# dimforge/salva

Hardware: AMD Instinct MI355X
Metric: particle-steps/sec (3D DFSPH) (higher is better)
Workload: dtype f32

## Files before the change

### bindings/rust/salva3d-hip/src/ffi.rs

```rust
#![allow(non_camel_case_types, non_snake_case, dead_code)]

#[repr(C)] pub struct SalvaHipWorld { _private: [u8; 0] }
#[repr(C)] pub struct SalvaHipComm { _private: [u8; 0] }
#[repr(C)] pub struct SalvaHipPeerSetup { _private: [u8; 0] }

pub const SALVA_HIP_OK: i32 = 0;
pub const SALVA_HIP_E_HIP: i32 = -1;
pub const SALVA_HIP_E_INVALID: i32 = -2;
pub const SALVA_HIP_E_NUMERIC: i32 = -3;
pub const SALVA_HIP_E_CAPACITY: i32 = -4;

pub const SALVA_HIP_SOLVER_DFSPH: i32 = 0;
pub const SALVA_HIP_SOLVER_IISPH: i32 = 1;

pub const SALVA_HIP_KERNEL_CUBIC_SPLINE: i32 = 0;
pub const SALVA_HIP_KERNEL_POLY6: i32 = 1;
pub const SALVA_HIP_KERNEL_SPIKY: i32 = 2;
pub const SALVA_HIP_KERNEL_VISCOSITY: i32 = 3;

pub const SALVA_HIP_FORCE_XSPH: i32 = 1;
pub const SALVA_HIP_FORCE_ARTIFICIAL: i32 = 2;
pub const SALVA_HIP_FORCE_AKINCI2013: i32 = 3;
pub const SALVA_HIP_FORCE_DFSPH_VISCOSITY: i32 = 4;
pub const SALVA_HIP_FORCE_HE2014: i32 = 5;
pub const SALVA_HIP_FORCE_WCSPH_TENSION: i32 = 6;
pub const SALVA_HIP_FORCE_CUSTOM: i32 = 7;
pub const SALVA_HIP_FORCE_BECKER2009: i32 = 8;
pub const SALVA_HIP_FORCE_DEVICE: i32 = 9;

pub const SALVA_HIP_DEVICE_NEEDS_FF: i32 = 1;
pub const SALVA_HIP_DEVICE_NEEDS_FB: i32 = 2;
pub const SALVA_HIP_DEVICE_NEEDS_KERNEL: i32 = 4;

pub const SALVA_HIP_DIRTY_POSITIONS: i32 = 1;
pub const SALVA_HIP_DIRTY_VELOCITIES: i32 = 2;
pub const SALVA_HIP_DIRTY_VOLUMES: i32 = 4;
pub const SALVA_HIP_DIRTY_ACCELERATIONS: i32 = 8;
pub const SALVA_HIP_DIRTY_ALL: i32 = 15;

pub const SALVA_HIP_FIELD_DENSITY: i32 = 0;
pub const SALVA_HIP_FIELD_ALPHA: i32 = 1;
pub const SALVA_HIP_FIELD_NUM_FLUID_CONTACTS: i32 = 2;
pub const SALVA_HIP_FIELD_NUM_BOUNDARY_CONTACTS: i32 = 3;
pub const SALVA_HIP_FIELD_VELOCITY_CHANGE: i32 = 4;
pub const SALVA_HIP_FIELD_PRESSURE: i32 = 5;
pub const SALVA_HIP_FIELD_VOLUME: i32 = 6;
pub const SALVA_HIP_FIELD_ACCELERATION: i32 = 7;

pub const SALVA_HIP_SHAPE_BALL: i32 = 1;
pub const SALVA_HIP_SHAPE_CUBOID: i32 = 2;
pub const SALVA_HIP_SHAPE_CAPSULE: i32 = 3;
pub const SALVA_HIP_SHAPE_CYLINDER: i32 = 4;
pub const SALVA_HIP_SHAPE_MESH: i32 = 5;
pub const SALVA_HIP_SHAPE_HOST: i32 = 100;

pub const SALVA_HIP_SAMPLE_SURFACE: i32 = 0;
pub const SALVA_HIP_SAMPLE_VOLUME: i32 = 1;

pub const SALVA_HIP_MESH_ORIENTED: i32 = 1;

pub const SALVA_HIP_SHAPE_COMPOUND: i32 = 6;

pub const SALVA_HIP_COMPOUND_MAX_PARTS: i32 = 64;

pub const SALVA_HIP_DEVICE_VIEW_VERSION: i32 = 1;
pub const SALVA_HIP_DEVICE_VIEW_BYTES: i32 = 240;
pub const SALVA_HIP_PEER_HANDLE_BYTES: i32 = 64;

#[repr(C)] #[derive(Clone, Copy, Debug)]
pub struct SalvaHipCounters_stages {
    pub collision_detection_time: f64,
    pub solver_time: f64,
}

#[repr(C)] #[derive(Clone, Copy, Debug)]
pub struct SalvaHipCounters_cd {
    pub ncontacts: u64,
    pub boundary_update_time: f64,
    pub grid_insertion_time: f64,
    pub neighborhood_search_time: f64,
    pub contact_sorting_time: f64,
}

#[repr(C)] #[derive(Clone, Copy, Debug)]
pub struct SalvaHipCounters_solver {
    pub non_pressure_resolution_time: f64,
    pub pressure_resolution_time: f64,
}

#[repr(C)] #[derive(Clone, Copy, Debug)]
pub struct SalvaHipParams {
    pub particle_radius: f32,
    pub smoothing_factor: f32,
    pub solver: i32,
    pub min_pressure_iter: i32,
    pub max_pressure_iter: i32,
    pub max_density_error: f32,
    pub min_divergence_iter: i32,
    pub max_divergence_iter: i32,
    pub max_divergence_error: f32,
    pub device: i32,
    pub enable_timers: i32,
    pub kernel_density: i32,
    pub kernel_gradient: i32,
    pub reserved: [i32; 5],
}

#[repr(C)] #[derive(Clone, Copy, Debug)]
pub struct SalvaHipForceDesc {
    pub kind: i32,
    pub p: [f32; 7],
}

#[repr(C)] #[derive(Clone, Copy, Debug)]
pub struct SalvaHipStepStats {
    pub n_divergence_iters: i32,
    pub n_pressure_iters: i32,
    pub divergence_error: f32,
    pub density_error: f32,
    pub ncontacts: u64,
    pub nparticles: u64,
    pub grid_ms: f32,
    pub solver_ms: f32,
    pub step_ms: f32,
    pub reserved: [f32; 5],
}

#[repr(C)] #[derive(Clone, Copy, Debug)]
pub struct SalvaHipCounters {
    pub nsubsteps: u64,
// ... 217 lines not shown
```

### include/salva_hip.h

```cpp
#ifndef SALVA_HIP_H
#define SALVA_HIP_H

#include <stdint.h>

#ifdef __cplusplus
extern "C" {
#endif

typedef struct SalvaHipWorld SalvaHipWorld;

enum {
    SALVA_HIP_OK = 0,
    SALVA_HIP_E_HIP = -1,
    SALVA_HIP_E_INVALID = -2,
    SALVA_HIP_E_NUMERIC = -3,
    SALVA_HIP_E_CAPACITY = -4
};

enum { SALVA_HIP_SOLVER_DFSPH = 0, SALVA_HIP_SOLVER_IISPH = 1 };
enum {
    SALVA_HIP_KERNEL_CUBIC_SPLINE = 0,
    SALVA_HIP_KERNEL_POLY6 = 1,
    SALVA_HIP_KERNEL_SPIKY = 2,
    SALVA_HIP_KERNEL_VISCOSITY = 3
// ... 16 lines not shown
    int32_t reserved[5];
} SalvaHipParams;

enum {
    SALVA_HIP_FORCE_XSPH = 1,
    SALVA_HIP_FORCE_ARTIFICIAL = 2,
    SALVA_HIP_FORCE_AKINCI2013 = 3,
    SALVA_HIP_FORCE_DFSPH_VISCOSITY = 4,
    SALVA_HIP_FORCE_HE2014 = 5,
    SALVA_HIP_FORCE_WCSPH_TENSION = 6,
    SALVA_HIP_FORCE_CUSTOM = 7,
    SALVA_HIP_FORCE_BECKER2009 = 8,
    SALVA_HIP_FORCE_DEVICE = 9
};
enum {
    SALVA_HIP_DEVICE_NEEDS_FF = 1,
    SALVA_HIP_DEVICE_NEEDS_FB = 2,
    SALVA_HIP_DEVICE_NEEDS_KERNEL = 4
};
typedef struct SalvaHipForceDesc {
    int32_t kind;
    float p[7];
} SalvaHipForceDesc;

enum {
    SALVA_HIP_DIRTY_POSITIONS = 1,
    SALVA_HIP_DIRTY_VELOCITIES = 2,
    SALVA_HIP_DIRTY_VOLUMES = 4,
    SALVA_HIP_DIRTY_ACCELERATIONS = 8,
    SALVA_HIP_DIRTY_ALL = 15
};

typedef struct SalvaHipStepStats {
    int32_t n_divergence_iters;
    int32_t n_pressure_iters;
    float divergence_error;
    float density_error;
    uint64_t ncontacts;
    uint64_t nparticles;
    float grid_ms;
    float solver_ms;
    float step_ms;
    float reserved[5];
} SalvaHipStepStats;

typedef struct SalvaHipCounters {
    uint64_t nsubsteps;
    double step_time;
    double custom;
    struct {
        double collision_detection_time;
        double solver_time;
    } stages;
    struct {
        uint64_t ncontacts;
        double boundary_update_time;
        double grid_insertion_time;
        double neighborhood_search_time;
        double contact_sorting_time;
    } cd;
    struct {
        double non_pressure_resolution_time;
        double pressure_resolution_time;
    } solver;
    int32_t n_divergence_iters, n_pressure_iters;
    uint64_t speculative_passes;
    uint64_t discarded_passes;
    uint64_t chained_passes;
    uint64_t chain_breaks;
    uint64_t pregrid_adopted;
    uint64_t pregrid_dropped;
    uint64_t light_class_passes;
    uint64_t sparse_class_passes;
} SalvaHipCounters;

enum {
    SALVA_HIP_FIELD_DENSITY = 0,
    SALVA_HIP_FIELD_ALPHA = 1,
    SALVA_HIP_FIELD_NUM_FLUID_CONTACTS = 2,
    SALVA_HIP_FIELD_NUM_BOUNDARY_CONTACTS = 3,
    SALVA_HIP_FIELD_VELOCITY_CHANGE = 4,
    SALVA_HIP_FIELD_PRESSURE = 5,
    SALVA_HIP_FIELD_VOLUME = 6,
    SALVA_HIP_FIELD_ACCELERATION = 7
};

void salva_hip_default_params(SalvaHipParams* out);

int salva_hip_create(const SalvaHipParams* params, SalvaHipWorld** out);
void salva_hip_destroy(SalvaHipWorld* world);

float salva_hip_h(const SalvaHipWorld* world);

int salva_hip_set_fluid(SalvaHipWorld* world, uint32_t slot, uint64_t n,
                        const float* positions_xyz, const float* velocities_xyz, const float* volumes,
                        const float* accelerations_xyz, const float* velocity_changes_xyz,
                        float density0, uint32_t memberships, uint32_t filter, uint32_t dirty_mask);

int salva_hip_set_fluid_forces(SalvaHipWorld* world, uint32_t slot, const SalvaHipForceDesc* forces, uint32_t nforces);

int salva_hip_remove_fluid(SalvaHipWorld* world, uint32_t slot);

int salva_hip_set_boundary(SalvaHipWorld* world, uint32_t slot, uint64_t n,
                           const float* positions_xyz, const float* velocities_xyz,
                           uint32_t memberships, uint32_t filter, int32_t wants_forces);
int salva_hip_remove_boundary(SalvaHipWorld* world, uint32_t slot);

uint32_t salva_hip_num_fluids(const SalvaHipWorld* world);
uint32_t salva_hip_num_boundaries(const SalvaHipWorld* world);
uint64_t salva_hip_fluid_len(const SalvaHipWorld* world, uint32_t slot);
uint64_t salva_hip_boundary_len(const SalvaHipWorld* world, uint32_t slot);

int salva_hip_step(SalvaHipWorld* world, float dt, const float gravity[3], SalvaHipStepStats* stats_or_null);

int salva_hip_get_fluid(SalvaHipWorld* world, uint32_t slot, float* positions_xyz, float* velocities_xyz);
int salva_hip_get_fluid_field(SalvaHipWorld* world, uint32_t slot, int32_t field, float* out);

typedef struct SalvaHipRigidPose {
    float translation[3];
    float rotation[4];
    float linvel[3];
    float angvel[3];
    float world_com[3];
    int32_t has_body;
    int32_t is_dynamic;
} SalvaHipRigidPose;

int salva_hip_set_boundary_sampling(SalvaHipWorld* world, uint32_t slot, uint64_t n, const float* local_points_xyz,
                                    uint32_t memberships, uint32_t filter);
int salva_hip_update_boundary_pose(SalvaHipWorld* world, uint32_t slot, const SalvaHipRigidPose* pose);
int salva_hip_update_boundary_poses(SalvaHipWorld* world, uint32_t n, const uint32_t* slots, const SalvaHipRigidPose* poses);
int salva_hip_get_boundary_particles(SalvaHipWorld* world, uint32_t slot, float* positions_xyz, float* velocities_xyz);
int salva_hip_get_boundary_wrench(SalvaHipWorld* world, uint32_t slot, const float point[3], float force[3], float torque[3]);
int salva_hip_get_boundary_wrenches(SalvaHipWorld* world, uint32_t n, const uint32_t* slots, const float* points_xyz, float* forces_xyz,
                                    float* torques_xyz);

typedef int (*SalvaHipForceCallback)(void* user, SalvaHipWorld* world, uint32_t fluid_slot, uint32_t force_index, float dt,
                                     float inv_dt);
int salva_hip_set_force_callback(SalvaHipWorld* world, SalvaHipForceCallback cb, void* user);
int salva_hip_force_get_state(SalvaHipWorld* world, uint32_t slot, float* positions_xyz, float* velocities_xyz, float* densities);
int salva_hip_force_add_accelerations(SalvaHipWorld* world, uint32_t slot, const float* accelerations_xyz);

#define SALVA_HIP_DEVICE_VIEW_VERSION 1
#define SALVA_HIP_DEVICE_VIEW_BYTES 240
typedef struct SalvaHipDeviceView {
    uint32_t struct_size;
    uint32_t version;
    void* stream;
    uint32_t fluid_slot, force_index;
    float dt, inv_dt;
    float h, particle_radius;
    int32_t kernel_density, kernel_gradient;
    float params[7];
    uint32_t needs;
    uint32_t n, nfluids;
    const float* posm;
    const float* vel;
    float* acc;
    const float* rho;
    const uint32_t* model;
    const uint32_t* id;
    const float* rho0;
    uint32_t nb;
    float bforce_scale;
    const float* bposv;
    const float* bvel;
    const uint32_t* bid;
// ... 192 lines not shown
```

### salva_amd/_lib.py

```python
from __future__ import annotations

import ctypes as C
import os
import subprocess

_HERE = os.path.dirname(os.path.abspath(__file__))
CSRC = os.path.join(_HERE, "csrc")
LIB_PATH = os.path.join(CSRC, "libsalva_hip.so")
if os.environ.get("SALVA_HIP_LIB_VARIANT"):
    LIB_PATH = os.path.join(CSRC, "libsalva_hip_%s.so" % os.environ["SALVA_HIP_LIB_VARIANT"])

OK, E_HIP, E_INVALID, E_NUMERIC, E_CAPACITY = 0, -1, -2, -3, -4
SOLVER_DFSPH, SOLVER_IISPH = 0, 1
(FORCE_XSPH, FORCE_ARTIFICIAL, FORCE_AKINCI2013, FORCE_DFSPH_VISCOSITY, FORCE_HE2014, FORCE_WCSPH_TENSION, FORCE_CUSTOM,
 FORCE_BECKER2009, FORCE_DEVICE) = 1, 2, 3, 4, 5, 6, 7, 8, 9
DEVICE_NEEDS_FF, DEVICE_NEEDS_FB, DEVICE_NEEDS_KERNEL = 1, 2, 4
DIRTY_POSITIONS, DIRTY_VELOCITIES, DIRTY_VOLUMES, DIRTY_ACCELERATIONS, DIRTY_ALL = 1, 2, 4, 8, 15
(FIELD_DENSITY, FIELD_ALPHA, FIELD_NUM_FLUID_CONTACTS, FIELD_NUM_BOUNDARY_CONTACTS, FIELD_VELOCITY_CHANGE,
 FIELD_PRESSURE, FIELD_VOLUME, FIELD_ACCELERATION) = range(8)

EXPORTED_SYMBOLS = [
    "salva_hip_default_params", "salva_hip_create", "salva_hip_destroy", "salva_hip_h", "salva_hip_set_fluid",
    "salva_hip_set_fluid_forces", "salva_hip_remove_fluid", "salva_hip_set_boundary", "salva_hip_remove_boundary",
    "salva_hip_num_fluids", "salva_hip_num_boundaries", "salva_hip_fluid_len", "salva_hip_boundary_len",
    "salva_hip_step", "salva_hip_get_fluid", "salva_hip_get_fluid_field", "salva_hip_get_boundary",
    "salva_hip_clear_boundary_forces", "salva_hip_device_bytes", "salva_hip_time_pred_density",
    "salva_hip_last_error", "salva_hip_version", "salva_hip_comm_rccl_unique_id", "salva_hip_comm_rccl_create",
    "salva_hip_comm_loopback_create", "salva_hip_comm_destroy", "salva_hip_set_domain", "salva_hip_get_owned",
    "salva_hip_get_force_stats", "salva_hip_get_fluid_contacts", "salva_hip_add_particles", "salva_hip_delete_particles",
    "salva_hip_particles_intersecting_aabb", "salva_hip_set_boundary_sampling", "salva_hip_update_boundary_pose",
    "salva_hip_get_boundary_particles", "salva_hip_get_boundary_wrench", "salva_hip_set_force_callback",
    "salva_hip_force_get_state", "salva_hip_force_add_accelerations", "salva_hip_set_fluid_field", "salva_hip_get_timestep",
    "salva_hip_set_timestep", "salva_hip_get_counters", "salva_hip_time_kernel", "salva_hip_particles_intersecting_shape", "salva_hip_rebalance",
    "salva_hip_set_boundary_dynamic_sampling", "salva_hip_get_boundary_sources", "salva_hip_set_boundary_dynamic_sampling_host",
    "salva_hip_delete_owned", "salva_hip_enable_counters", "salva_hip_comm_peer_begin", "salva_hip_comm_peer_connect",
    "salva_hip_comm_peer_abort", "salva_hip_comm_selftest", "salva_hip_comm_time", "salva_hip_clear_boundary_sampling", "salva_hip_get_fluid_async", "salva_hip_wait_download",
    "salva_hip_host_alloc", "salva_hip_host_free", "salva_hip_host_register", "salva_hip_host_unregister",
    "salva_hip_set_cfl", "salva_hip_get_substeps", "salva_hip_particles_intersecting_host_shape",
    "salva_hip_set_coupling_callback", "salva_hip_get_tile_tables",
    "salva_hip_get_dist_timing", "salva_hip_local_len", "salva_hip_get_local", "salva_hip_get_local_contacts", "salva_hip_force_add_local_accelerations",
    "salva_hip_get_elasticity_state", "salva_hip_set_elasticity_state", "salva_hip_get_elasticity_contacts",
    "salva_hip_sample_shape", "salva_hip_sample_host_shape", "salva_hip_add_particles_sampled", "salva_hip_set_boundary_sampling_from_shape",
    "salva_hip_create_mesh", "salva_hip_create_heightfield", "salva_hip_destroy_mesh", "salva_hip_sample_mesh",
    "salva_hip_add_particles_sampled_mesh", "salva_hip_set_boundary_sampling_from_mesh", "salva_hip_set_boundary_dynamic_sampling_mesh",
    "salva_hip_update_boundary_poses", "salva_hip_get_boundary_wrenches", "salva_hip_get_dcs_stats",
    "salva_hip_set_device_force_callback", "salva_hip_device_view_read", "salva_hip_get_device_force_stats",
    "salva_hip_create_compound", "salva_hip_destroy_compound", "salva_hip_set_boundary_dynamic_sampling_compound",
    "salva_hip_particles_intersecting_compound", "salva_hip_particles_intersecting_mesh",
    "salva_hip_sample_compound", "salva_hip_add_particles_sampled_compound", "salva_hip_set_boundary_sampling_from_compound",
]


class Params(C.Structure):
    _fields_ = [
        ("particle_radius", C.c_float),
        ("smoothing_factor", C.c_float),
        ("solver", C.c_int32),
        ("min_pressure_iter", C.c_int32),
        ("max_pressure_iter", C.c_int32),
        ("max_density_error", C.c_float),
        ("min_divergence_iter", C.c_int32),
        ("max_divergence_iter", C.c_int32),
        ("max_divergence_error", C.c_float),
        ("device", C.c_int32),
        ("enable_timers", C.c_int32),
        ("kernel_density", C.c_int32),
        ("kernel_gradient", C.c_int32),
        ("reserved", C.c_int32 * 5),
    ]


class ForceDesc(C.Structure):
    _fields_ = [("kind", C.c_int32), ("p", C.c_float * 7)]


FORCE_CALLBACK = C.CFUNCTYPE(C.c_int, C.c_void_p, C.c_void_p, C.c_uint32, C.c_uint32, C.c_float, C.c_float)
COUPLING_CALLBACK = C.CFUNCTYPE(C.c_int, C.c_void_p, C.c_void_p, C.c_int32, C.c_float)


class DeviceView(C.Structure):
    _fields_ = [("struct_size", C.c_uint32), ("version", C.c_uint32),
                ("stream", C.c_void_p), ("fluid_slot", C.c_uint32), ("force_index", C.c_uint32), ("dt", C.c_float), ("inv_dt", C.c_float),
                ("h", C.c_float), ("particle_radius", C.c_float), ("kernel_density", C.c_int32), ("kernel_gradient", C.c_int32),
                ("params", C.c_float * 7), ("needs", C.c_uint32),
                ("n", C.c_uint32), ("nfluids", C.c_uint32), ("posm", C.c_void_p), ("vel", C.c_void_p), ("acc", C.c_void_p),
                ("rho", C.c_void_p), ("model", C.c_void_p), ("id", C.c_void_p), ("rho0", C.c_void_p),
                ("nb", C.c_uint32), ("bforce_scale", C.c_float), ("bposv", C.c_void_p), ("bvel", C.c_void_p), ("bid", C.c_void_p),
                ("bforce_fx", C.c_void_p), ("bwants", C.c_void_p),
                ("ff_off", C.c_void_p), ("ff_j", C.c_void_p), ("fb_off", C.c_void_p), ("fb_j", C.c_void_p),
                ("ff_kern", C.c_void_p), ("fb_kern", C.c_void_p)]


DEVICE_VIEW_BYTES, DEVICE_VIEW_VERSION = 240, 1
DEVICE_FORCE_CALLBACK = C.CFUNCTYPE(C.c_int, C.c_void_p, C.c_void_p, C.POINTER(DeviceView))


class RigidPose(C.Structure):
    _fields_ = [("translation", C.c_float * 3), ("rotation", C.c_float * 4), ("linvel", C.c_float * 3),
                ("angvel", C.c_float * 3), ("world_com", C.c_float * 3), ("has_body", C.c_int32), ("is_dynamic", C.c_int32)]


class StepStats(C.Structure):
# ... 260 lines not shown
```

### salva_amd/csrc/device_types.h

```cpp
#pragma once
#include <hip/hip_runtime.h>

#include <cstdint>

#include "sph_math.h"

namespace salva {

struct TileGrid {
    int ox, oy, oz;
    int ntx, nty, ntz;
    uint32_t mx, my, mz;
    const uint32_t* cell_start;
};

struct TileAcc {
    uint64_t s;
    uint64_t sb;
    uint32_t nsl;
    uint32_t nonempty;
    uint32_t max_s, max_sb, max_nsl;
    uint32_t max_sum;
    uint32_t max_raw;
    uint32_t wsl;
// ... 21 lines not shown

struct TileListStats { uint32_t sum_ff, sum_fb, max_ff, max_fb, own_ff, own_fb, ref_s, ref_sb; };

struct PrePub { int32_t on, chained; int32_t bbox[6]; };

struct StepCtx {
    SphConsts sc;
    uint32_t xcd;

    uint32_t n;
    float4* posm;
    float4* vel;
    float4* dv;
    float4* acc;
    float4* w;
    float4* normal;
    uint32_t* model;
    uint32_t* perm;
    const uint32_t* gtag;
    float* rho;
    float* alpha;
    float* kappa;
    float* kappa2;
    float* rho_star;
    float* aii;
    float4* dii;
    float4* dijpj;
    float4* posmr;
    float4* iisph_q;
    float4* iisph_pr;
    uint32_t* nff;
    uint32_t* nfb;
    uint32_t* nbr_ff;
    uint32_t* nbr_fb;
    uint32_t* slice_near;
    uint32_t cap_ff, cap_fb;
    const TileAcc* tile_off;
    const uint32_t* halo_src;
    const uint32_t* bhalo_src;
    uint32_t halo_stride;
    uint32_t bhalo_stride;
    uint32_t ntiles;
    uint32_t split_s;
    const uint32_t* tile_ids;
    const uint4* slot_desc;
    const uint4* slot_info;
    const uint32_t* tile_rank;
    const uint32_t* slot_order;
    uint32_t slot_base;
    uint32_t ntiny;
    uint32_t nlight;
    uint32_t nlaunch;
    uint32_t spec;
    uint32_t halo_cap, bhalo_cap;
    uint32_t nslices_cap;
    uint64_t halo_len, bhalo_len;
    TileGrid gf;
    const uint32_t* stale_keys;

    uint32_t nb;
    float4* bposv;
    float4* bvel;
    uint32_t* bperm;
    float4* bforce;
    unsigned long long* bforce_fx;
    float bforce_scale;
    const uint8_t* bwants;
    TileGrid gb;

    uint32_t nmodels, nbmodels;
    const float* rho0_tab;
    float rho0_single;
    float mass_uniform;
    uint32_t* tile_mass_bits;
    uint32_t* tile_massb_bits;
    uint2* tile_masscd_bits;
    uint32_t* nffb;
    uint32_t* nffc;
    uint32_t two_mass;
    uint32_t nmass;
    uint64_t cmask;
    float class_mass[4];
    uint32_t bvel_zero;
    const uint8_t* ff_ok;
    const uint8_t* fb_ok;
    const uint8_t* bb_ok;

    float* partials;
    int spec_k;
    uint32_t spec_external;
    SolveCtl* spec_ring;
    SolveCtl* spec_pub;
    const uint32_t* model_counts;
    float4* w2;
    uint32_t* flags;
    uint32_t min_neighbors_for_divergence;
    int32_t phase, ghost_lo_cx, ghost_hi_cx;
    const SolveCtl* ctl;
    const uint32_t* gate;
    uint32_t gate_stage;
#ifdef SALVA_HIP_DIAG
    unsigned long long* dbg;
#endif
};

constexpr uint32_t MASS_SLOTS = 64;

struct Readback {
    float err;
    uint32_t flags;
    int32_t bbox[6];
    int32_t bbbox[6];
    TileAcc tile_total;
    uint64_t ncontacts_bb;
    uint64_t ncontacts_ff, ncontacts_fb;
    uint32_t max_cnt_ff, max_cnt_fb;
    uint32_t dcs_count;
    uint32_t cfl_max_bits;
    uint64_t ncontacts_own_ff, ncontacts_own_fb;
    uint32_t mass_mm[2];
    uint32_t pad2_[2];
    uint32_t chain_ok, chain_stage;
    uint32_t solve[2][4];
    uint32_t pre_ok;
    uint32_t max_ref[3];
};
#ifdef __HIPCC__
__device__ __forceinline__ bool gate_words_closed(uint32_t ok, uint32_t stage, uint32_t my_stage) { return ok == 0u && !(my_stage != 0u && stage == my_stage); }
__device__ __forceinline__ bool gate_closed(const StepCtx& c) { return c.gate && gate_words_closed(c.gate[0], c.gate[1], c.gate_stage); }
#endif

}
```

### salva_amd/csrc/dfsph.hip

```cpp
#include <climits>

#include "bbox.h"
#include "kernels.h"
#include "tile.h"

namespace SALVA_KNS {
using namespace salva;

unsigned num_blocks(uint32_t n) { return div_up(n, BLOCK); }

}
#include "pairs.h"
namespace SALVA_KNS {
using namespace salva;

static inline bool plane_layouts(const StepCtx& c) { return c.mass_uniform > 0.0f || c.two_mass != 0u; }

#ifndef SALVA_DA_IISPH_WAVES
#define SALVA_DA_IISPH_WAVES 6
#endif
template <bool IISPH>
__global__ __launch_bounds__(TILE_MAX_THREADS, IISPH ? SALVA_DA_IISPH_WAVES : 1) void k_density_alpha(StepCtx c, float dt) {
    lds_base_check();
    Tile t;
// ... 8 lines not shown
    t.stage(c, static_cast<const float4*>(c.posm), Lp);
    const float4* Bp = nullptr;
    t.stage_boundary(c, Bp);
    Tile::staged_barrier();
    t.for_own_pre(own0, load_own, [&](const Own& o, uint32_t i, uint32_t gs, bool active) {
        const uint32_t nqu = slice_list_dwords(o.cnt, active);
        const float4 pi = o.pi;
        float rho = 0.0f, gsx = 0.0f, gsy = 0.0f, gsz = 0.0f, sq = 0.0f;
        uint32_t nnear = 0;
        if (active) {
            f2 rw = {0.0f, 0.0f}, ax = {0.0f, 0.0f}, ay = {0.0f, 0.0f}, az = {0.0f, 0.0f}, s2 = {0.0f, 0.0f};
            const f2 tiny = {1.0e-30f, 1.0e-30f};
            for_each_ff2<true, false, true>(c, gs, nqu, o.lh, [&](uint32_t off) { return lds_ld16(off); }, [&](const float4& A, const float4& B) { SALVA_PAIR_MATH
                const f2 dx = {pi.x - A.x, pi.x - B.x}, dy = {pi.y - A.y, pi.y - B.y}, dz = {pi.z - A.z, pi.z - B.z};
                f2 r2 = dz * dz + tiny;
                r2 = dy * dy + r2;
                r2 = dx * dx + r2;
                const bool za = r2.x <= c.sc.tiny_r2, zb = r2.y <= c.sc.tiny_r2;
                nnear += (za ? 1u : 0u) + (zb ? 1u : 0u);
                const KernelWG2 k = kernel_wg2(r2, c.sc);
                const f2 m = {A.w, B.w};
                f2 wm = k.w * m;
                wm.x = za ? 0.0f : wm.x; wm.y = zb ? 0.0f : wm.y;
                rw += wm;
                const f2 gm = k.g * m;
                ax += dx * gm; ay += dy * gm; az += dz * gm;
                if (!IISPH) s2 += (gm * gm) * r2;
                else s2 += (k.g * gm) * r2;
            });
            const uint32_t npad = 2u * nqu - o.cnt;
            rho = (rw.x + rw.y) * c.sc.wscale + pi.w * c.sc.wnorm;
            gsx = (ax.x + ax.y) * c.sc.gscale; gsy = (ay.x + ay.y) * c.sc.gscale; gsz = (az.x + az.y) * c.sc.gscale;
            sq = (s2.x + s2.y) * (c.sc.gscale * c.sc.gscale);
            nnear -= npad;
        }
#ifdef SALVA_OTHER_KERNELS
        const bool any_near = __builtin_amdgcn_ballot_w64(active && nnear > 1u) != 0ull || (c.sc.kd | c.sc.kg) != 0;
#else
        const bool any_near = __builtin_amdgcn_ballot_w64(active && nnear > 1u) != 0ull;
#endif
        if (any_near && active) {
            rho = gsx = gsy = gsz = sq = 0.0f;
            for_each_ff(c, i, gs, [&](uint32_t s) { SALVA_PAIR_MATH
                const float4 pj = lds_ld16(s << 4);
                const float dx = pi.x - pj.x, dy = pi.y - pj.y, dz = pi.z - pj.z;
                const KernelEval e = kernel_eval(dx * dx + dy * dy + dz * dz, c.sc);
                rho += pj.w * e.w;
                const float gm = e.g * pj.w;
                const float gx = dx * gm, gy = dy * gm, gz = dz * gm;
                if (!IISPH) sq += gx * gx + gy * gy + gz * gz;
                else sq += (dx * e.g) * gx + (dy * e.g) * gy + (dz * e.g) * gz;
                gsx += gx; gsy += gy; gsz += gz;
            });
        }
        if (active) {
            const float rho0 = rho0_of(c, o.mi);
            for_each_fb(c, t, i, gs, [&](uint32_t s) { SALVA_PAIR_MATH
                const float4 pj = Bp[s];
                const float dx = pi.x - pj.x, dy = pi.y - pj.y, dz = pi.z - pj.z;
                const KernelEval e = kernel_eval(dx * dx + dy * dy + dz * dz, c.sc);
                const float m = pj.w * rho0;
                rho += m * e.w;
                const float gm = e.g * m;
                const float gx = dx * gm, gy = dy * gm, gz = dz * gm;
                if (!IISPH) sq += gx * gx + gy * gy + gz * gz;
                else sq += (dx * e.g) * gx + (dy * e.g) * gy + (dz * e.g) * gz;
                gsx += gx; gsy += gy; gsz += gz;
            });
            if (!(rho > 0.0f)) atomicOr(c.flags, 1u);
            c.rho[i] = rho;
            if (IISPH) {
                const float f0 = dt * dt / (rho * rho);
                const float dxi = -(gsx * f0), dyi = -(gsy * f0), dzi = -(gsz * f0);
                c.dii[i] = make_float4(dxi, dyi, dzi, 0.0f);
                c.aii[i] = (dxi * gsx + dyi * gsy + dzi * gsz) - (f0 * pi.w) * sq;
                c.kappa[i] = c.dv[i].w * 0.5f;
                c.iisph_pr[i] = make_float4(pi.x, pi.y, pi.z, pi.w / (rho * rho));
            } else {
                const float denom = sq + (gsx * gsx + gsy * gsy + gsz * gsz);
                c.alpha[i] = (denom <= 1.0e-5f) ? 0.0f : 1.0f / denom;
            }
            c.posmr[i] = make_float4(pi.x, pi.y, pi.z, pi.w / rho);
        }
        if ((threadIdx.x & (WAVE - 1)) == 0) c.slice_near[gs] = any_near ? 1u : 0u;
    });
}
void launch_density_alpha(const StepCtx& c, const TileLds& L, float iisph_dt, hipStream_t s) {
    SALVA_OK_DISPATCH(launch_density_alpha, c, L, iisph_dt, s);
    if (iisph_dt > 0.0f) SALVA_LAUNCH_TILE(k_density_alpha<true>, c, L, L.bytes(16, 16, 2), s, c, iisph_dt);
    else SALVA_LAUNCH_TILE(k_density_alpha<false>, c, L, L.bytes(16, 16, 2), s, c, 0.0f);
}

#ifndef SALVA_DAD_WAVES
#define SALVA_DAD_WAVES 5
#endif
template <uint32_t DS, int TWO>
__device__ __forceinline__ void k_density_alpha_div_p3_body(StepCtx c) {
    lds_base_check();
    Tile t;
    t.setup(c);
    if (t.empty()) { TileErr::zero(c, t.slot); return; }
    struct Own { float px, py, pz, ux, uy, uz; uint32_t cnt; ListRegs lh; };
    auto load_own = [&](uint32_t i, uint32_t gs) {
        const float4 p = c.posm[i], u = c.w[i];
        return Own{p.x, p.y, p.z, u.x, u.y, u.z, c.nff[i], list_regs(c, gs)};
    };
    uint32_t i0, gs0;
    t.first_own(i0, gs0);
    const Own own0 = load_own(i0, gs0);
    const uint32_t dist8 = p3_dist8<DS>(t);
    t.stage_p3(c, static_cast<const float4*>(c.posm), static_cast<const float4*>(c.w), dist8);
    const float4* Bp = nullptr;
    t.stage_boundary(c, Bp);
    TileErrC E;
    E.init(reinterpret_cast<float*>(t.pool + t.pool_used), c);
    Tile::staged_barrier();
    const float m = t.mass;
    t.for_own_pre(own0, load_own, [&](const Own& o, uint32_t i, uint32_t gs, bool active) {
        const uint32_t nqu = slice_list_dwords(o.cnt, active);
        const float3 pi = make_float3(o.px, o.py, o.pz), wi = make_float3(o.ux, o.uy, o.uz);
        float rho = 0.0f, gsx = 0.0f, gsy = 0.0f, gsz = 0.0f, sq = 0.0f, div = 0.0f;
        uint32_t nnear = 0;
        if (active) {
            f2 rw = {0.0f, 0.0f}, ax = {0.0f, 0.0f}, ay = {0.0f, 0.0f}, az = {0.0f, 0.0f}, s2 = {0.0f, 0.0f}, dv2 = {0.0f, 0.0f};
            const f2 tiny = {1.0e-30f, 1.0e-30f};
            for_each_ff2<true, false, 2>(c, gs, nqu, o.lh, [&](uint32_t off) { return load_p3(off, dist8); }, [&](const RecP3& A, const RecP3& B) { SALVA_PAIR_MATH
                const f2 dx = {pi.x - A.xy.x, pi.x - B.xy.x}, dy = {pi.y - A.xy.y, pi.y - B.xy.y}, dz = {pi.z - A.zu.x, pi.z - B.zu.x};
                f2 r2 = dz * dz + tiny;
                r2 = dy * dy + r2;
                r2 = dx * dx + r2;
                const bool za = r2.x <= c.sc.tiny_r2, zb = r2.y <= c.sc.tiny_r2;
                nnear += (za ? 1u : 0u) + (zb ? 1u : 0u);
                const KernelWG2 k = kernel_wg2(r2, c.sc);
                f2 wm = k.w;
                wm.x = za ? 0.0f : wm.x; wm.y = zb ? 0.0f : wm.y;
                rw += wm;
                ax += dx * k.g; ay += dy * k.g; az += dz * k.g;
                s2 += (k.g * k.g) * r2;
                const f2 ux = {wi.x - A.zu.y, wi.x - B.zu.y}, uy = {wi.y - A.vw.x, wi.y - B.vw.x}, uz = {wi.z - A.vw.y, wi.z - B.vw.y};
                dv2 += (ux * dx + uy * dy + uz * dz) * k.g;
            });
            const uint32_t npad = 2u * nqu - o.cnt;
            const float gm = c.sc.gscale * m;
            rho = (rw.x + rw.y) * c.sc.wscale * m + c.posm[i].w * c.sc.wnorm;
            gsx = (ax.x + ax.y) * gm; gsy = (ay.x + ay.y) * gm; gsz = (az.x + az.y) * gm;
            sq = (s2.x + s2.y) * (gm * gm);
            div = (dv2.x + dv2.y) * gm;
            nnear -= npad;
        }
        const bool any_near = __builtin_amdgcn_ballot_w64(active && nnear > 1u) != 0ull;
        if (any_near && active) {
            rho = gsx = gsy = gsz = sq = div = 0.0f;
            for_each_ff(c, i, gs, [&](uint32_t s) { SALVA_PAIR_MATH
                const RecP3 A = load_p3(s << 3, dist8);
                const float dx = pi.x - A.xy.x, dy = pi.y - A.xy.y, dz = pi.z - A.zu.x;
                const KernelEval e = kernel_eval(dx * dx + dy * dy + dz * dz, c.sc);
                rho += m * e.w;
                const float gmj = e.g * m;
                const float gx = dx * gmj, gy = dy * gmj, gz = dz * gmj;
                sq += gx * gx + gy * gy + gz * gz;
                gsx += gx; gsy += gy; gsz += gz;
                div += ((wi.x - A.zu.y) * dx + (wi.y - A.vw.x) * dy + (wi.z - A.vw.y) * dz) * gmj;
            });
        }
        if (active && (TWO && t.massb != 0.0f)) {
            auto on_top = [&](uint32_t first, uint32_t last, float mold, float mnew) {
                float rwb = 0.0f, gxb = 0.0f, gyb = 0.0f, gzb = 0.0f, s2b = 0.0f, dvb = 0.0f;
                for_each_ff_range(c, gs, first, last, [&](uint32_t s) { SALVA_PAIR_MATH
                    const RecP3 A = load_p3(s << 3, dist8);
                    const float dx = pi.x - A.xy.x, dy = pi.y - A.xy.y, dz = pi.z - A.zu.x;
                    const float r2 = dx * dx + dy * dy + dz * dz;
                    const KernelEval e = kernel_eval(r2, c.sc);
                    if (any_near || r2 > c.sc.tiny_r2) rwb += e.w;
                    const float gx = dx * e.g, gy = dy * e.g, gz = dz * e.g;
                    gxb += gx; gyb += gy; gzb += gz;
                    s2b += gx * gx + gy * gy + gz * gz;
                    dvb += ((wi.x - A.zu.y) * dx + (wi.y - A.vw.x) * dy + (wi.z - A.vw.y) * dz) * e.g;
                });
                const float dm = mnew - mold;
                rho += dm * rwb; gsx += dm * gxb; gsy += dm * gyb; gsz += dm * gzb;
                sq += (mnew * mnew - mold * mold) * s2b;
                div += dm * dvb;
            };
            const uint32_t nb2 = c.nffb[i];
            if (nb2) on_top(o.cnt - nb2, o.cnt, m, t.massb);
            if (TWO == 2 && t.massc != 0.0f) {
                const uint32_t cd = c.nffc[i], l2 = cd & 0xffffu, l3 = cd >> 16;
                if (l2) on_top(o.cnt - l3 - l2, o.cnt - l3, t.massb, t.massc);
                if (l3) on_top(o.cnt - l3, o.cnt, t.massb, t.massd);
            }
        }
        float err = 0.0f;
        uint32_t mi = 0;
        if (active) {
            mi = c.model[i];
            const float rho0 = rho0_of(c, mi);
            for_each_fb(c, t, i, gs, [&](uint32_t s) { SALVA_PAIR_MATH
                const float4 pj = Bp[s];
                const float dx = pi.x - pj.x, dy = pi.y - pj.y, dz = pi.z - pj.z;
                const KernelEval e = kernel_eval(dx * dx + dy * dy + dz * dz, c.sc);
                const float mb = pj.w * rho0;
                rho += mb * e.w;
                const float gmb = e.g * mb;
                const float gx = dx * gmb, gy = dy * gmb, gz = dz * gmb;
                sq += gx * gx + gy * gy + gz * gz;
                gsx += gx; gsy += gy; gsz += gz;
                div += (wi.x * dx + wi.y * dy + wi.z * dz) * gmb;
            });
            if (!(rho > 0.0f)) atomicOr(c.flags, 1u);
            const float denom = sq + (gsx * gsx + gsy * gsy + gsz * gsz);
            const float alpha = (denom <= 1.0e-5f) ? 0.0f : 1.0f / denom;
            c.rho[i] = rho;
            c.alpha[i] = alpha;
            c.posmr[i] = make_float4(pi.x, pi.y, pi.z, c.posm[i].w / rho);
            const uint32_t cntb = c.nb ? c.nfb[i] : 0u;
            div = (o.cnt + cntb >= c.min_neighbors_for_divergence) ? fmaxf(div, 0.0f) : 0.0f;
            c.kappa[i] = div * alpha;
            err = div / rho0;
        }
        if ((threadIdx.x & (WAVE - 1)) == 0) c.slice_near[gs] = any_near ? 1u : 0u;
        E.add(c, err, mi, active && !is_ghost(c, i));
    });
    E.finish(c, t.slot);
}
template <uint32_t DS>
__global__ __launch_bounds__(TILE_MAX_THREADS, (DS) == P3_DS_THREE ? SALVA_DAD_WAVES : 5) void k_density_alpha_div_p3(StepCtx c) { k_density_alpha_div_p3_body<DS, 0>(c); }
template <uint32_t DS>
__global__ __launch_bounds__(TILE_MAX_THREADS, (DS) == P3_DS_THREE ? SALVA_DAD_WAVES : 5) void k_density_alpha_div_p3_two(StepCtx c) { k_density_alpha_div_p3_body<DS, 1>(c); }
template <uint32_t DS>
__global__ __launch_bounds__(TILE_MAX_THREADS, (DS) == P3_DS_THREE ? SALVA_DAD_WAVES : 5) void k_density_alpha_div_p3_multi(StepCtx c) { k_density_alpha_div_p3_body<DS, 2>(c); }
bool launch_density_alpha_div(const StepCtx& c, const TileLds& L, hipStream_t s) {
#ifndef SALVA_OTHER_KERNELS
    if (!plane_layouts(c) || (c.sc.kd | c.sc.kg) != 0) return false;
    const uint32_t ds = pick_ds_p3(L.max_halo_fluid, L.ds_level);
    if (c.two_mass && c.nmass > 2u) SALVA_LAUNCH_P3(k_density_alpha_div_p3_multi, ds, c, L, p3_bytes(L, ds, c.nmodels, false), s, c);
    else if (c.two_mass) SALVA_LAUNCH_P3(k_density_alpha_div_p3_two, ds, c, L, p3_bytes(L, ds, c.nmodels, false), s, c);
    else SALVA_LAUNCH_P3(k_density_alpha_div_p3, ds, c, L, p3_bytes(L, ds, c.nmodels, false), s, c);
    return true;
#else
    return false;
#endif
}

__device__ __forceinline__ const SolveCtl* solve_record(const StepCtx& c) { return c.spec_k >= 0 ? c.spec_ring + (c.spec_k & 1) : c.ctl; }
__device__ __forceinline__ const float4* solve_w_in(const StepCtx& c, const SolveCtl* r) {
    return (c.spec_k >= 0 && (r->iters & 1u)) ? c.w2 : c.w;
}
__device__ __forceinline__ void spec_decide(const StepCtx& c, float* scratch) {
    typedef uint32_t u32x4 __attribute__((ext_vector_type(4)));
    const SolveCtl* rk = c.spec_ring + (c.spec_k & 1);
    SolveCtl* rn = c.spec_ring + ((c.spec_k + 1) & 1);
    const u32x4 c0 = reinterpret_cast<const u32x4*>(rk)[0], c1 = reinterpret_cast<const u32x4*>(rk)[1];
    const uint32_t done = c0.x, iters = c0.y, seq = c0.w + 1u, min_iter = c1.y;
    const float tol = __uint_as_float(c1.x);
    u32x4 out = {1u, iters, c0.z, seq};
    if (!done) {
        float best = 0.0f;
        const uint32_t nb = c.nlaunch, nm = c.nmodels;
        for (uint32_t m = 0; m < nm; ++m) {
            for (uint32_t v = threadIdx.x; v < 1024u; v += blockDim.x) {
                float s = 0.0f;
                for (uint32_t b = v; b < nb; b += 1024u) s += c.partials[(size_t)b * nm + m];
                s = wave_sum(s);
                if ((v & 63u) == 0u) scratch[v >> 6] = s;
            }
            __syncthreads();
            if (threadIdx.x == 0) {
                float tot = 0.0f;
                for (int k = 0; k < 16; ++k) tot += scratch[k];
                const uint32_t cnt = c.model_counts[m];
                if (cnt != 0) best = fmaxf(best, tot / (float)cnt);
            }
            __syncthreads();
        }
        const bool ok = best <= tol && iters >= min_iter;
        out = u32x4{ok ? 1u : 0u, ok ? iters : iters + 1u, __float_as_uint(best), seq};
    }
    if (threadIdx.x == 0) {
        reinterpret_cast<u32x4*>(rn)[0] = out;
        reinterpret_cast<u32x4*>(rn)[1] = c1;
        if (c.spec_pub) *reinterpret_cast<volatile u32x4*>(c.spec_pub) = out;
    }
}

template <uint32_t DS>
__global__ __launch_bounds__(TILE_MAX_THREADS) void k_divergence(StepCtx c) {
    const SolveCtl* const rec = solve_record(c);
    if (rec && rec->done) return;
    const float4* const win = rec ? solve_w_in(c, rec) : c.w;
    lds_base_check();
    Tile t;
    t.setup(c);
    if (t.skipped()) return;
    if (t.empty()) { TileErr::zero(c, t.slot); return; }
    struct Own { float4 pi, wi; float alpha; uint32_t mi, cnt, cntb, near; ListRegs lh; };
    auto load_own = [&](uint32_t i, uint32_t gs) {
        return Own{c.posm[i], win[i], c.alpha[i], c.model[i], c.nff[i], c.nb ? c.nfb[i] : 0u, c.slice_near[gs], list_regs(c, gs)};
    };
    uint32_t i0, gs0;
    t.first_own(i0, gs0);
    const Own own0 = load_own(i0, gs0);
    const uint32_t dist = pw_dist<DS>(c, t);
    const float4* Bp = nullptr;
    const float4* Bv = nullptr;
    t.stage_pw(c, static_cast<const float4*>(c.posm), win, dist, Bp, Bv, false);
    TileErr E;
    E.init(carve_errtab(t), c);
    Tile::staged_barrier();
    t.for_own_pre(own0, load_own, [&](const Own& o, uint32_t i, uint32_t gs, bool active) {
        const uint32_t nqu = slice_list_dwords(o.cnt, active);
        const bool near = slice_is_near(c, o.near);
        float err = 0.0f;
        uint32_t mi = 0;
        if (active) {
            mi = o.mi;
            const float rho0 = rho0_of(c, mi);
            float div = 0.0f;
            if (o.cnt + o.cntb >= c.min_neighbors_for_divergence) {
                const float4 pi = o.pi, wi = o.wi;
                div += near ? pair_sum_velocity_divergence_exact(c, i, gs, pi, wi, dist)
                            : pair_sum_velocity_divergence(c, gs, nqu, o.lh, pi, wi, dist);
                for_each_fb(c, t, i, gs, [&](uint32_t s) { SALVA_PAIR_MATH
                    const float4 pj = Bp[s];
                    const float dx = pi.x - pj.x, dy = pi.y - pj.y, dz = pi.z - pj.z;
                    const float g = kernel_grad(dx * dx + dy * dy + dz * dz, c.sc);
                    div += (wi.x * dx + wi.y * dy + wi.z * dz) * g * (pj.w * rho0);
                });
                div = fmaxf(div, 0.0f);
            }
            c.kappa[i] = div * o.alpha;
            err = div / rho0;
        }
        E.add(c, err, mi, active && !is_ghost(c, i));
    });
    E.finish(c, t.slot);
}
#define SALVA_P3_BOUNDS(DS) __launch_bounds__(TILE_MAX_THREADS, (DS) == P3_DS_THREE ? 6 : 5)
#ifndef SALVA_EVAL_POST
#define SALVA_EVAL_POST false
#endif
template <uint32_t DS, int TWO>
__device__ __forceinline__ void k_divergence_p3_body(StepCtx c) {
    const SolveCtl* const rec = solve_record(c);
    if (rec && rec->done) return;
    const float4* const win = rec ? solve_w_in(c, rec) : c.w;
    lds_base_check();
    Tile t;
    t.setup(c);
    if (t.skipped()) return;
    if (t.empty()) { TileErr::zero(c, t.slot); return; }
    constexpr bool POST = TWO || SALVA_EVAL_POST;
    struct Own { float px, py, pz, ux, uy, uz, alpha; uint32_t mi, cnt, cntb, nb2, near; ListRegs lh; };
    auto load_own = [&](uint32_t i, uint32_t gs) {
        const float4 p = c.posm[i], u = win[i];
        return Own{p.x, p.y, p.z, u.x, u.y, u.z, POST ? 0.0f : c.alpha[i], POST ? 0u : c.model[i], c.nff[i], c.nb ? c.nfb[i] : 0u,
                   (TWO && t.massb != 0.0f) ? c.nffb[i] : 0u, c.slice_near[gs], list_regs(c, gs)};
    };
    uint32_t i0, gs0;
    t.first_own(i0, gs0);
    const Own own0 = load_own(i0, gs0);
    const uint32_t dist8 = p3_dist8<DS>(t);
    t.stage_p3(c, static_cast<const float4*>(c.posm), win, dist8);
    const float4* Bp = nullptr;
    t.stage_boundary(c, Bp);
    TileErrC E;
    E.init(reinterpret_cast<float*>(t.pool + t.pool_used), c);
    Tile::staged_barrier();
    t.for_own_pre(own0, load_own, [&](const Own& o, uint32_t i, uint32_t gs, bool active) {
        const uint32_t nqu = slice_list_dwords(o.cnt, active);
        const bool near = slice_is_near(c, o.near);
        float err = 0.0f;
        uint32_t mi = 0;
        if (active) {
            mi = POST ? c.model[i] : o.mi;
            const float rho0 = rho0_of(c, mi);
            float div = 0.0f;
            if (o.cnt + o.cntb >= c.min_neighbors_for_divergence) {
                const float4 pi = make_float4(o.px, o.py, o.pz, 0.0f), wi = make_float4(o.ux, o.uy, o.uz, 0.0f);
                if ((TWO && t.massb != 0.0f) && !near) {
                    div += pair_sum_velocity_divergence_p3_two(c, gs, nqu, o.lh, pi, wi, dist8, o.cnt - o.nb2, t.mass, t.massb);
                } else {
                    div += near ? pair_sum_velocity_divergence_exact_p3(c, i, gs, pi, wi, dist8, t.mass)
                                : pair_sum_velocity_divergence_p3(c, gs, nqu, o.lh, pi, wi, dist8, t.mass);
                    if ((TWO && t.massb != 0.0f) && o.nb2)
                        div += (t.massb - t.mass) * pair_tail_velocity_divergence_p3(c, gs, o.cnt - o.nb2, o.cnt, pi, wi, dist8);
                }
                if (TWO == 2 && t.massc != 0.0f) {
                    const uint32_t cd = c.nffc[i], l2 = cd & 0xffffu, l3 = cd >> 16;
                    if (l2) div += (t.massc - t.massb) * pair_tail_velocity_divergence_p3(c, gs, o.cnt - l3 - l2, o.cnt - l3, pi, wi, dist8);
                    if (l3) div += (t.massd - t.massb) * pair_tail_velocity_divergence_p3(c, gs, o.cnt - l3, o.cnt, pi, wi, dist8);
                }
                for_each_fb(c, t, i, gs, [&](uint32_t s) { SALVA_PAIR_MATH
                    const float4 pj = Bp[s];
                    const float dx = pi.x - pj.x, dy = pi.y - pj.y, dz = pi.z - pj.z;
                    const float g = kernel_grad(dx * dx + dy * dy + dz * dz, c.sc);
                    div += (wi.x * dx + wi.y * dy + wi.z * dz) * g * (pj.w * rho0);
                });
                div = fmaxf(div, 0.0f);
            }
            c.kappa[i] = div * (POST ? c.alpha[i] : o.alpha);
            err = div / rho0;
        }
        E.add(c, err, mi, active && !is_ghost(c, i));
    });
    E.finish(c, t.slot);
}
template <uint32_t DS>
__global__ SALVA_P3_BOUNDS(DS) void k_divergence_p3(StepCtx c) { k_divergence_p3_body<DS, 0>(c); }
template <uint32_t DS>
__global__ SALVA_P3_BOUNDS(DS) void k_divergence_p3_two(StepCtx c) { k_divergence_p3_body<DS, 1>(c); }
template <uint32_t DS>
__global__ SALVA_P3_BOUNDS(DS) void k_divergence_p3_multi(StepCtx c) { k_divergence_p3_body<DS, 2>(c); }
void launch_divergence(const StepCtx& c, const TileLds& L, hipStream_t s) {
    SALVA_OK_DISPATCH(launch_divergence, c, L, s);
    if (plane_layouts(c)) {
        const uint32_t ds = pick_ds_p3(L.max_halo_fluid, L.ds_level);
        if (c.two_mass && c.nmass > 2u) SALVA_LAUNCH_P3(k_divergence_p3_multi, ds, c, L, p3_bytes(L, ds, c.nmodels, false), s, c);
        else if (c.two_mass) SALVA_LAUNCH_P3(k_divergence_p3_two, ds, c, L, p3_bytes(L, ds, c.nmodels, false), s, c);
        else SALVA_LAUNCH_P3(k_divergence_p3, ds, c, L, p3_bytes(L, ds, c.nmodels, false), s, c);
        return;
    }
    const uint32_t ds = pick_ds(pw_slots(L), L.ds_level);
    SALVA_LAUNCH_FIXED(k_divergence, ds, c, L, pw_bytes(L, ds, true), s, c);
}

template <uint32_t DS>
__global__ __launch_bounds__(TILE_MAX_THREADS) void k_divergence_apply(StepCtx c, float inv_dt_prev) {
    const SolveCtl* const rec = solve_record(c);
    const bool was_done = rec && rec->done;
    const float4* const win = rec ? solve_w_in(c, rec) : c.w;
    float4* const wout = c.spec_k >= 0 ? ((win == c.w) ? c.w2 : c.w) : c.w;
    lds_base_check();
    if (c.spec_k >= 0 && !c.spec_external && blockIdx.x == 0 && c.slot_base == 0u) {
        spec_decide(c, reinterpret_cast<float*>(tile_smem));
        __syncthreads();
    }
    if (was_done) return;
    Tile t;
    t.setup(c);
    if (t.empty()) return;
    struct Own { float4 pi, wi; float ki; uint32_t cnt, near; ListRegs lh; };
    auto load_own = [&](uint32_t i, uint32_t gs) {
        return Own{c.posm[i], win[i], c.kappa[i], c.nff[i], c.slice_near[gs], list_regs(c, gs)};
    };
    uint32_t i0, gs0;
    t.first_own(i0, gs0);
    const Own own0 = load_own(i0, gs0);
    const uint32_t dist = pk_dist<DS>(c, t);
    const float4* Bp = nullptr;
    const float4* Bv = nullptr;
    t.stage_pk(c, static_cast<const float4*>(c.posm), static_cast<const float*>(c.kappa), dist, Bp, Bv);
    Tile::staged_barrier();
    t.for_own_pre(own0, load_own, [&](const Own& o, uint32_t i, uint32_t gs, bool active) {
        const uint32_t nqu = slice_list_dwords(o.cnt, active);
        const bool near = slice_is_near(c, o.near);
        if (!active) return;
        const float4 pi = o.pi;
        const uint32_t mi = __float_as_uint(o.wi.w);
        const float rho0 = rho0_of(c, mi);
        const float ki = o.ki;
        float4 d = o.wi;
        float sx, sy, sz;
        if (near) pair_sum_gradient_exact(c, i, gs, pi, dist, [&](float kj) { return ki + kj; }, sx, sy, sz);
        else pair_sum_gradient(c, gs, nqu, o.lh, pi, dist, [&](float ka, float kb) { return f2{ki + ka, ki + kb}; }, sx, sy, sz);
        d.x -= sx; d.y -= sy; d.z -= sz;
        for_each_fb(c, t, i, gs, [&](uint32_t s) { SALVA_PAIR_MATH
            const float4 pj = Bp[s];
            const float dx = pi.x - pj.x, dy = pi.y - pj.y, dz = pi.z - pj.z;
            const float g = kernel_grad(dx * dx + dy * dy + dz * dz, c.sc);
            const float coeff = -ki * pj.w * rho0 * g;
            const float ex = dx * coeff, ey = dy * coeff, ez = dz * coeff;
            d.x += ex; d.y += ey; d.z += ez;
            if (c.bforce && !is_ghost(c, i)) {
                const float fs = -inv_dt_prev * pi.w;
                apply_boundary_force(c, boundary_sorted_of_slot(c, t, s), __float_as_uint(Bv[s].w), ex * fs, ey * fs, ez * fs);
            }
        });
        wout[i] = d;
    });
}
#ifndef SALVA_P2_WAVES
#define SALVA_P2_WAVES 6
#endif
#define SALVA_P2_BOUNDS(DS) __launch_bounds__(TILE_MAX_THREADS, (DS) == P2_DS_THREE ? SALVA_P2_WAVES : 5)
template <uint32_t DS, int TWO>
__device__ __forceinline__ void k_divergence_apply_p2_body(StepCtx c, float inv_dt_prev) {
    const SolveCtl* const rec = solve_record(c);
    const bool was_done = rec && rec->done;
    const float4* const win = rec ? solve_w_in(c, rec) : c.w;
    float4* const wout = c.spec_k >= 0 ? ((win == c.w) ? c.w2 : c.w) : c.w;
    lds_base_check();
    if (c.spec_k >= 0 && !c.spec_external && blockIdx.x == 0 && c.slot_base == 0u) {
        spec_decide(c, reinterpret_cast<float*>(tile_smem));
        __syncthreads();
    }
    if (was_done) return;
    Tile t;
    t.setup(c);
    if (t.empty()) return;
    struct Own { float px, py, pz, ki; uint32_t cnt, nb2, near; ListRegs lh; };
    auto load_own = [&](uint32_t i, uint32_t gs) {
        const float4 p = c.posm[i];
        return Own{p.x, p.y, p.z, c.kappa[i], c.nff[i], (TWO && t.massb != 0.0f) ? c.nffb[i] : 0u, c.slice_near[gs], list_regs(c, gs)};
    };
    uint32_t i0, gs0;
    t.first_own(i0, gs0);
    const Own own0 = load_own(i0, gs0);
    const uint32_t dist8 = p2_dist8<DS>(t);
    t.stage_p2(c, static_cast<const float4*>(c.posm), static_cast<const float*>(c.kappa), dist8);
    Tile::staged_barrier();
    t.for_own_pre(own0, load_own, [&](const Own& o, uint32_t i, uint32_t gs, bool active) {
        const uint32_t nqu = slice_list_dwords(o.cnt, active);
        const bool near = slice_is_near(c, o.near);
        if (!active) return;
        const float4 pi = make_float4(o.px, o.py, o.pz, 0.0f);
        const float ki = o.ki;
        float sx, sy, sz;
        if ((TWO && t.massb != 0.0f) && !near) {
            pair_sum_gradient_p2_two(c, gs, nqu, o.lh, pi, dist8, o.cnt - o.nb2, t.mass, t.massb, [&](float ka, float kb) { return f2{ki + ka, ki + kb}; }, sx, sy, sz);
        } else {
            if (near) pair_sum_gradient_exact_p2(c, i, gs, pi, dist8, t.mass, [&](float kj) { return ki + kj; }, sx, sy, sz);
            else pair_sum_gradient_p2(c, gs, nqu, o.lh, pi, dist8, t.mass, [&](float ka, float kb) { return f2{ki + ka, ki + kb}; }, sx, sy, sz);
            if ((TWO && t.massb != 0.0f) && o.nb2) {
                float bx, by, bz;
                pair_tail_gradient_p2(c, gs, o.cnt - o.nb2, o.cnt, pi, dist8, [&](float kj) { return ki + kj; }, bx, by, bz);
                const float dm = t.massb - t.mass;
                sx += dm * bx; sy += dm * by; sz += dm * bz;
            }
        }
        if (TWO == 2 && t.massc != 0.0f) {
            const uint32_t cd = c.nffc[i], l2 = cd & 0xffffu, l3 = cd >> 16;
            float bx, by, bz;
            if (l2) {
                pair_tail_gradient_p2(c, gs, o.cnt - l3 - l2, o.cnt - l3, pi, dist8, [&](float kj) { return ki + kj; }, bx, by, bz);
                const float dm = t.massc - t.massb;
                sx += dm * bx; sy += dm * by; sz += dm * bz;
            }
            if (l3) {
                pair_tail_gradient_p2(c, gs, o.cnt - l3, o.cnt, pi, dist8, [&](float kj) { return ki + kj; }, bx, by, bz);
                const float dm = t.massd - t.massb;
                sx += dm * bx; sy += dm * by; sz += dm * bz;
            }
        }
        float4 d = win[i];
        const uint32_t mi = __float_as_uint(d.w);
        const float rho0 = rho0_of(c, mi);
        d.x -= sx; d.y -= sy; d.z -= sz;
        for_each_fb(c, t, i, gs, [&](uint32_t s) { SALVA_PAIR_MATH
            const float4 pj = p2_boundary_pos(t, s, dist8);
            const float dx = pi.x - pj.x, dy = pi.y - pj.y, dz = pi.z - pj.z;
            const float g = kernel_grad(dx * dx + dy * dy + dz * dz, c.sc);
            const float coeff = -ki * pj.w * rho0 * g;
            const float ex = dx * coeff, ey = dy * coeff, ez = dz * coeff;
            d.x += ex; d.y += ey; d.z += ez;
            if (c.bforce && !is_ghost(c, i)) {
                const float fs = -inv_dt_prev * c.posm[i].w;
                const uint32_t jb = boundary_sorted_of_slot(c, t, s);
                apply_boundary_force(c, jb, __float_as_uint(c.bvel[jb].w), ex * fs, ey * fs, ez * fs);
            }
        });
        wout[i] = d;
    });
}
template <uint32_t DS>
__global__ SALVA_P2_BOUNDS(DS) void k_divergence_apply_p2(StepCtx c, float inv_dt_prev) { k_divergence_apply_p2_body<DS, 0>(c, inv_dt_prev); }
template <uint32_t DS>
__global__ SALVA_P2_BOUNDS(DS) void k_divergence_apply_p2_two(StepCtx c, float inv_dt_prev) { k_divergence_apply_p2_body<DS, 1>(c, inv_dt_prev); }
template <uint32_t DS>
__global__ SALVA_P2_BOUNDS(DS) void k_divergence_apply_p2_multi(StepCtx c, float inv_dt_prev) { k_divergence_apply_p2_body<DS, 2>(c, inv_dt_prev); }
void launch_divergence_apply(const StepCtx& c, const TileLds& L, float inv_dt_prev, hipStream_t s) {
    SALVA_OK_DISPATCH(launch_divergence_apply, c, L, inv_dt_prev, s);
    if (plane_layouts(c)) {
        const uint32_t ds = pick_ds_p2(L.raw_slots(), L.ds_level);
        if (c.two_mass && c.nmass > 2u) SALVA_LAUNCH_P2(k_divergence_apply_p2_multi, ds, c, L, p2_bytes(L, ds), s, c, inv_dt_prev);
        else if (c.two_mass) SALVA_LAUNCH_P2(k_divergence_apply_p2_two, ds, c, L, p2_bytes(L, ds), s, c, inv_dt_prev);
        else SALVA_LAUNCH_P2(k_divergence_apply_p2, ds, c, L, p2_bytes(L, ds), s, c, inv_dt_prev);
        return;
    }
    const uint32_t ds = pick_ds(pk_slots(L), L.ds_level);
    SALVA_LAUNCH_FIXED(k_divergence_apply, ds, c, L, pk_bytes(L, ds), s, c, inv_dt_prev);
}

__global__ __launch_bounds__(BLOCK) void k_finish_divergence(StepCtx c, float gx, float gy, float gz, int acc_has_user) {
    const uint32_t i = blockIdx.x * BLOCK + threadIdx.x;
    if (i >= c.n || gate_closed(c)) return;
    const float4 wi = c.w[i];
    const float4 v = c.vel[i];
    const float4 d = c.dv[i];
    c.vel[i] = make_float4(wi.x, wi.y, wi.z, v.w);
    c.dv[i] = make_float4(0.0f, 0.0f, 0.0f, d.w);
    float4 a = make_float4(0.0f, 0.0f, 0.0f, 0.0f);
    if (acc_has_user) a = c.acc[i];
    c.acc[i] = make_float4(a.x + gx, a.y + gy, a.z + gz, 0.0f);
}
void launch_finish_divergence(const StepCtx& c, float gx, float gy, float gz, bool acc_has_user, hipStream_t s) {
    if (c.n) k_finish_divergence<<<num_blocks(c.n), BLOCK, 0, s>>>(c, gx, gy, gz, acc_has_user ? 1 : 0);
}

__global__ __launch_bounds__(BLOCK) void k_integrate(StepCtx c, float dt) {
    const uint32_t i = blockIdx.x * BLOCK + threadIdx.x;
    if (i >= c.n || gate_closed(c)) return;
    const float4 a = c.acc[i];
    float4 d = c.dv[i];
    d.x += a.x * dt; d.y += a.y * dt; d.z += a.z * dt;
    c.dv[i] = d;
    c.acc[i] = make_float4(0.0f, 0.0f, 0.0f, 0.0f);
    const float4 v = c.vel[i];
    c.w[i] = make_float4(v.x + d.x, v.y + d.y, v.z + d.z, __uint_as_float(c.model[i]));
}
void launch_integrate(const StepCtx& c, float dt, hipStream_t s) {
    if (c.n) k_integrate<<<num_blocks(c.n), BLOCK, 0, s>>>(c, dt);
}

#ifdef SALVA_HIP_DIAG
#define SALVA_DIAG_STAMP(name) const unsigned long long name = __builtin_readcyclecounter()
#else
#define SALVA_DIAG_STAMP(name)
#endif
template <uint32_t DS>
__global__ __launch_bounds__(TILE_MAX_THREADS) void k_pred_density(StepCtx c, float dt) {
    if (c.ctl && c.ctl->done) return;
    lds_base_check();
    SALVA_DIAG_STAMP(T0);
    Tile t;
    t.setup(c);
    if (t.skipped()) return;
    if (t.empty()) { TileErr::zero(c, t.slot); return; }
    SALVA_DIAG_STAMP(T1);
    struct Own { float4 pi, wi; float rho, alpha; uint32_t mi, cnt, near; ListRegs lh; };
    auto load_own = [&](uint32_t i, uint32_t gs) {
        return Own{c.posm[i], c.w[i], c.rho[i], c.alpha[i], c.model[i], c.nff[i], c.slice_near[gs], list_regs(c, gs)};
    };
    uint32_t i0, gs0;
    t.first_own(i0, gs0);
    const Own own0 = load_own(i0, gs0);
    const uint32_t dist = pw_dist<DS>(c, t);
    const float4* Bp = nullptr;
    const float4* Bv = nullptr;
    t.stage_pw(c, static_cast<const float4*>(c.posm), static_cast<const float4*>(c.w), dist, Bp, Bv, true);
    TileErr E;
    E.init(carve_errtab(t), c);
    SALVA_DIAG_STAMP(T2);
    Tile::staged_barrier();
    SALVA_DIAG_STAMP(T3);
    t.for_own_pre(own0, load_own, [&](const Own& o, uint32_t i, uint32_t gs, bool active) {
        const uint32_t nqu = slice_list_dwords(o.cnt, active);
        const bool near = slice_is_near(c, o.near);
        float err = 0.0f;
        uint32_t mi = 0;
        if (active) {
            mi = o.mi;
            const float rho0 = rho0_of(c, mi);
            const float4 pi = o.pi, wi = o.wi;
            float delta = near ? pair_sum_velocity_divergence_exact(c, i, gs, pi, wi, dist)
                               : pair_sum_velocity_divergence(c, gs, nqu, o.lh, pi, wi, dist);
            for_each_fb(c, t, i, gs, [&](uint32_t s) { SALVA_PAIR_MATH
                const float4 pj = Bp[s];
                const float4 vj = Bv[s];
                const float dx = pi.x - pj.x, dy = pi.y - pj.y, dz = pi.z - pj.z;
                const float g = kernel_grad(dx * dx + dy * dy + dz * dz, c.sc);
                delta += pj.w * rho0 * (((wi.x - vj.x) * dx + (wi.y - vj.y) * dy + (wi.z - vj.z) * dz) * g);
            });
            const float rs = o.rho + delta * dt;
            if (!(rs != 0.0f)) atomicOr(c.flags, 1u);
            err = (rs < rho0) ? 0.0f : rs / rho0 - 1.0f;
            c.kappa[i] = (rs - rho0) * o.alpha;
        }
        E.add(c, err, mi, active && !is_ghost(c, i));
    });
    SALVA_DIAG_STAMP(T4);
    E.finish(c, t.slot);
#ifdef SALVA_HIP_DIAG
    if (c.dbg && threadIdx.x == 0) {
        unsigned long long* d = c.dbg + (size_t)t.slot * 8;
        d[0] = T0; d[1] = T1; d[2] = T2; d[3] = T3; d[4] = T4; d[5] = __builtin_readcyclecounter(); d[6] = t.S; d[7] = t.own_end - t.own_begin;
    }
#endif
}
template <uint32_t DS, int TWO>
__device__ __forceinline__ void k_pred_density_p3_body(StepCtx c, float dt) {
    if (c.ctl && c.ctl->done) return;
    lds_base_check();
    Tile t;
    t.setup(c);
    if (t.skipped()) return;
    if (t.empty()) { TileErr::zero(c, t.slot); return; }
    constexpr bool POST = TWO || SALVA_EVAL_POST;
    struct Own { float px, py, pz, ux, uy, uz, rho, alpha; uint32_t mi, cnt, nb2, near; ListRegs lh; };
    auto load_own = [&](uint32_t i, uint32_t gs) {
        const float4 p = c.posm[i], u = c.w[i];
        return Own{p.x, p.y, p.z, u.x, u.y, u.z, POST ? 0.0f : c.rho[i], POST ? 0.0f : c.alpha[i], POST ? 0u : c.model[i], c.nff[i],
                   (TWO && t.massb != 0.0f) ? c.nffb[i] : 0u, c.slice_near[gs], list_regs(c, gs)};
    };
    uint32_t i0, gs0;
    t.first_own(i0, gs0);
    const Own own0 = load_own(i0, gs0);
    const uint32_t dist8 = p3_dist8<DS>(t);
    t.stage_p3(c, static_cast<const float4*>(c.posm), static_cast<const float4*>(c.w), dist8);
    const float4* Bp = nullptr;
    const float4* Bv = nullptr;
    if (c.bvel_zero) t.stage_boundary(c, Bp);
    else t.stage_boundary(c, Bp, Bv);
    TileErrC E;
    E.init(reinterpret_cast<float*>(t.pool + t.pool_used), c);
    Tile::staged_barrier();
    t.for_own_pre(own0, load_own, [&](const Own& o, uint32_t i, uint32_t gs, bool active) {
        const uint32_t nqu = slice_list_dwords(o.cnt, active);
        const bool near = slice_is_near(c, o.near);
        float err = 0.0f;
        uint32_t mi = 0;
        if (active) {
            const float4 pi = make_float4(o.px, o.py, o.pz, 0.0f), wi = make_float4(o.ux, o.uy, o.uz, 0.0f);
            float delta;
            if ((TWO && t.massb != 0.0f) && !near) {
                delta = pair_sum_velocity_divergence_p3_two(c, gs, nqu, o.lh, pi, wi, dist8, o.cnt - o.nb2, t.mass, t.massb);
            } else {
                delta = near ? pair_sum_velocity_divergence_exact_p3(c, i, gs, pi, wi, dist8, t.mass)
                             : pair_sum_velocity_divergence_p3(c, gs, nqu, o.lh, pi, wi, dist8, t.mass);
                if ((TWO && t.massb != 0.0f) && o.nb2)
                    delta += (t.massb - t.mass) * pair_tail_velocity_divergence_p3(c, gs, o.cnt - o.nb2, o.cnt, pi, wi, dist8);
            }
            if (TWO == 2 && t.massc != 0.0f) {
                const uint32_t cd = c.nffc[i], l2 = cd & 0xffffu, l3 = cd >> 16;
                if (l2) delta += (t.massc - t.massb) * pair_tail_velocity_divergence_p3(c, gs, o.cnt - l3 - l2, o.cnt - l3, pi, wi, dist8);
                if (l3) delta += (t.massd - t.massb) * pair_tail_velocity_divergence_p3(c, gs, o.cnt - l3, o.cnt, pi, wi, dist8);
            }
            mi = POST ? c.model[i] : o.mi;
            const float rho0 = rho0_of(c, mi);
            for_each_fb(c, t, i, gs, [&](uint32_t s) { SALVA_PAIR_MATH
                const float4 pj = Bp[s];
                const float4 vj = c.bvel_zero ? make_float4(0.0f, 0.0f, 0.0f, 0.0f) : Bv[s];
                const float dx = pi.x - pj.x, dy = pi.y - pj.y, dz = pi.z - pj.z;
                const float g = kernel_grad(dx * dx + dy * dy + dz * dz, c.sc);
                delta += pj.w * rho0 * (((wi.x - vj.x) * dx + (wi.y - vj.y) * dy + (wi.z - vj.z) * dz) * g);
            });
            const float rs = (POST ? c.rho[i] : o.rho) + delta * dt;
            if (!(rs != 0.0f)) atomicOr(c.flags, 1u);
            err = (rs < rho0) ? 0.0f : rs / rho0 - 1.0f;
            c.kappa[i] = (rs - rho0) * (POST ? c.alpha[i] : o.alpha);
        }
        E.add(c, err, mi, active && !is_ghost(c, i));
    });
    E.finish(c, t.slot);
}
template <uint32_t DS>
__global__ SALVA_P3_BOUNDS(DS) void k_pred_density_p3(StepCtx c, float dt) { k_pred_density_p3_body<DS, 0>(c, dt); }
template <uint32_t DS>
__global__ SALVA_P3_BOUNDS(DS) void k_pred_density_p3_two(StepCtx c, float dt) { k_pred_density_p3_body<DS, 1>(c, dt); }
template <uint32_t DS>
__global__ SALVA_P3_BOUNDS(DS) void k_pred_density_p3_multi(StepCtx c, float dt) { k_pred_density_p3_body<DS, 2>(c, dt); }
void launch_pred_density(const StepCtx& c, const TileLds& L, float dt, hipStream_t s) {
    SALVA_OK_DISPATCH(launch_pred_density, c, L, dt, s);
    if (plane_layouts(c)) {
        const uint32_t ds = pick_ds_p3(L.max_halo_fluid, L.ds_level);
        if (c.two_mass && c.nmass > 2u) SALVA_LAUNCH_P3(k_pred_density_p3_multi, ds, c, L, p3_bytes(L, ds, c.nmodels, !c.bvel_zero), s, c, dt);
        else if (c.two_mass) SALVA_LAUNCH_P3(k_pred_density_p3_two, ds, c, L, p3_bytes(L, ds, c.nmodels, !c.bvel_zero), s, c, dt);
        else SALVA_LAUNCH_P3(k_pred_density_p3, ds, c, L, p3_bytes(L, ds, c.nmodels, !c.bvel_zero), s, c, dt);
        return;
    }
    const uint32_t ds = pick_ds(pw_slots(L), L.ds_level);
    SALVA_LAUNCH_FIXED(k_pred_density, ds, c, L, pw_bytes(L, ds, true), s, c, dt);
}

template <uint32_t DS>
__global__ __launch_bounds__(TILE_MAX_THREADS) void k_pressure_apply(StepCtx c, float inv_dt) {
    if (c.ctl && c.ctl->done) return;
    lds_base_check();
    Tile t;
    t.setup(c);
    if (t.empty()) return;
    struct Own { float4 pi, d, v; float ki; uint32_t mi, cnt, near; ListRegs lh; };
    auto load_own = [&](uint32_t i, uint32_t gs) {
        return Own{c.posm[i], c.dv[i], c.vel[i], c.kappa[i], c.model[i], c.nff[i], c.slice_near[gs], list_regs(c, gs)};
    };
    uint32_t i0, gs0;
    t.first_own(i0, gs0);
    const Own own0 = load_own(i0, gs0);
    const uint32_t dist = pk_dist<DS>(c, t);
    const float4* Bp = nullptr;
    const float4* Bv = nullptr;
    t.stage_pk(c, static_cast<const float4*>(c.posm), static_cast<const float*>(c.kappa), dist, Bp, Bv);
    Tile::staged_barrier();
    t.for_own_pre(own0, load_own, [&](const Own& o, uint32_t i, uint32_t gs, bool active) {
        const uint32_t nqu = slice_list_dwords(o.cnt, active);
        const bool near = slice_is_near(c, o.near);
        if (!active) return;
        const float4 pi = o.pi;
        const uint32_t mi = o.mi;
        const float rho0 = rho0_of(c, mi);
        const float ki = o.ki;
        const float kip = fmaxf(ki, 0.0f);
        float4 d = o.d;
        float sx, sy, sz;
        if (near) pair_sum_gradient_exact(c, i, gs, pi, dist, [&](float kj) { return kip + fmaxf(kj, 0.0f); }, sx, sy, sz);
        else pair_sum_gradient(c, gs, nqu, o.lh, pi, dist, [&](float ka, float kb) { return f2{kip + fmaxf(ka, 0.0f), kip + fmaxf(kb, 0.0f)}; }, sx, sy, sz);
        d.x -= sx * inv_dt; d.y -= sy * inv_dt; d.z -= sz * inv_dt;
        if (ki > 0.0f) {
            for_each_fb(c, t, i, gs, [&](uint32_t s) { SALVA_PAIR_MATH
                const float4 pj = Bp[s];
                const float dx = pi.x - pj.x, dy = pi.y - pj.y, dz = pi.z - pj.z;
                const float g = kernel_grad(dx * dx + dy * dy + dz * dz, c.sc);
                const float coeff = ki * pj.w * rho0 * inv_dt * g;
                const float ex = dx * coeff, ey = dy * coeff, ez = dz * coeff;
                d.x -= ex; d.y -= ey; d.z -= ez;
                if (c.bforce && !is_ghost(c, i)) {
                    const float fs = inv_dt * pi.w;
                    apply_boundary_force(c, boundary_sorted_of_slot(c, t, s), __float_as_uint(Bv[s].w), ex * fs, ey * fs, ez * fs);
                }
            });
        }
        c.dv[i] = d;
        const float4 v = o.v;
        c.w[i] = make_float4(v.x + d.x, v.y + d.y, v.z + d.z, __uint_as_float(mi));
    });
}
template <uint32_t DS, int TWO>
__device__ __forceinline__ void k_pressure_apply_p2_body(StepCtx c, float inv_dt) {
    if (c.ctl && c.ctl->done) return;
    lds_base_check();
    Tile t;
    t.setup(c);
    if (t.empty()) return;
    struct Own { float px, py, pz, ki; uint32_t cnt, nb2, near; ListRegs lh; };
    auto load_own = [&](uint32_t i, uint32_t gs) {
        const float4 p = c.posm[i];
        return Own{p.x, p.y, p.z, c.kappa[i], c.nff[i], (TWO && t.massb != 0.0f) ? c.nffb[i] : 0u, c.slice_near[gs], list_regs(c, gs)};
    };
    uint32_t i0, gs0;
    t.first_own(i0, gs0);
    const Own own0 = load_own(i0, gs0);
    const uint32_t dist8 = p2_dist8<DS>(t);
    t.stage_p2(c, static_cast<const float4*>(c.posm), static_cast<const float*>(c.kappa), dist8);
    Tile::staged_barrier();
    t.for_own_pre(own0, load_own, [&](const Own& o, uint32_t i, uint32_t gs, bool active) {
        const uint32_t nqu = slice_list_dwords(o.cnt, active);
        const bool near = slice_is_near(c, o.near);
        if (!active) return;
        const float4 pi = make_float4(o.px, o.py, o.pz, 0.0f);
        const float ki = o.ki;
        const float kip = fmaxf(ki, 0.0f);
        float sx, sy, sz;
        if ((TWO && t.massb != 0.0f) && !near) {
            pair_sum_gradient_p2_two(c, gs, nqu, o.lh, pi, dist8, o.cnt - o.nb2, t.mass, t.massb,
                                     [&](float ka, float kb) { return f2{kip + fmaxf(ka, 0.0f), kip + fmaxf(kb, 0.0f)}; }, sx, sy, sz);
        } else {
            if (near) pair_sum_gradient_exact_p2(c, i, gs, pi, dist8, t.mass, [&](float kj) { return kip + fmaxf(kj, 0.0f); }, sx, sy, sz);
            else pair_sum_gradient_p2(c, gs, nqu, o.lh, pi, dist8, t.mass, [&](float ka, float kb) { return f2{kip + fmaxf(ka, 0.0f), kip + fmaxf(kb, 0.0f)}; }, sx, sy, sz);
            if ((TWO && t.massb != 0.0f) && o.nb2) {
                float bx, by, bz;
                pair_tail_gradient_p2(c, gs, o.cnt - o.nb2, o.cnt, pi, dist8, [&](float kj) { return kip + fmaxf(kj, 0.0f); }, bx, by, bz);
                const float dm = t.massb - t.mass;
                sx += dm * bx; sy += dm * by; sz += dm * bz;
            }
        }
        if (TWO == 2 && t.massc != 0.0f) {
            const uint32_t cd = c.nffc[i], l2 = cd & 0xffffu, l3 = cd >> 16;
            float bx, by, bz;
            if (l2) {
                pair_tail_gradient_p2(c, gs, o.cnt - l3 - l2, o.cnt - l3, pi, dist8, [&](float kj) { return kip + fmaxf(kj, 0.0f); }, bx, by, bz);
                const float dm = t.massc - t.massb;
                sx += dm * bx; sy += dm * by; sz += dm * bz;
            }
            if (l3) {
                pair_tail_gradient_p2(c, gs, o.cnt - l3, o.cnt, pi, dist8, [&](float kj) { return kip + fmaxf(kj, 0.0f); }, bx, by, bz);
                const float dm = t.massd - t.massb;
                sx += dm * bx; sy += dm * by; sz += dm * bz;
            }
        }
        const uint32_t mi = c.model[i];
        const float rho0 = rho0_of(c, mi);
        float4 d = c.dv[i];
        d.x -= sx * inv_dt; d.y -= sy * inv_dt; d.z -= sz * inv_dt;
        if (ki > 0.0f) {
            for_each_fb(c, t, i, gs, [&](uint32_t s) { SALVA_PAIR_MATH
                const float4 pj = p2_boundary_pos(t, s, dist8);
                const float dx = pi.x - pj.x, dy = pi.y - pj.y, dz = pi.z - pj.z;
                const float g = kernel_grad(dx * dx + dy * dy + dz * dz, c.sc);
                const float coeff = ki * pj.w * rho0 * inv_dt * g;
                const float ex = dx * coeff, ey = dy * coeff, ez = dz * coeff;
                d.x -= ex; d.y -= ey; d.z -= ez;
                if (c.bforce && !is_ghost(c, i)) {
                    const float fs = inv_dt * c.posm[i].w;
                    const uint32_t jb = boundary_sorted_of_slot(c, t, s);
                    apply_boundary_force(c, jb, __float_as_uint(c.bvel[jb].w), ex * fs, ey * fs, ez * fs);
                }
            });
        }
        c.dv[i] = d;
        const float4 v = c.vel[i];
        c.w[i] = make_float4(v.x + d.x, v.y + d.y, v.z + d.z, __uint_as_float(mi));
    });
}
template <uint32_t DS>
__global__ SALVA_P2_BOUNDS(DS) void k_pressure_apply_p2(StepCtx c, float inv_dt) { k_pressure_apply_p2_body<DS, 0>(c, inv_dt); }
template <uint32_t DS>
__global__ SALVA_P2_BOUNDS(DS) void k_pressure_apply_p2_two(StepCtx c, float inv_dt) { k_pressure_apply_p2_body<DS, 1>(c, inv_dt); }
template <uint32_t DS>
__global__ SALVA_P2_BOUNDS(DS) void k_pressure_apply_p2_multi(StepCtx c, float inv_dt) { k_pressure_apply_p2_body<DS, 2>(c, inv_dt); }
void launch_pressure_apply(const StepCtx& c, const TileLds& L, float inv_dt, hipStream_t s) {
    SALVA_OK_DISPATCH(launch_pressure_apply, c, L, inv_dt, s);
    if (plane_layouts(c)) {
        const uint32_t ds = pick_ds_p2(L.raw_slots(), L.ds_level);
        if (c.two_mass && c.nmass > 2u) SALVA_LAUNCH_P2(k_pressure_apply_p2_multi, ds, c, L, p2_bytes(L, ds), s, c, inv_dt);
        else if (c.two_mass) SALVA_LAUNCH_P2(k_pressure_apply_p2_two, ds, c, L, p2_bytes(L, ds), s, c, inv_dt);
        else SALVA_LAUNCH_P2(k_pressure_apply_p2, ds, c, L, p2_bytes(L, ds), s, c, inv_dt);
        return;
    }
    const uint32_t ds = pick_ds(pk_slots(L), L.ds_level);
    SALVA_LAUNCH_FIXED(k_pressure_apply, ds, c, L, pk_bytes(L, ds), s, c, inv_dt);
}

__global__ __launch_bounds__(BLOCK) void k_update_positions(StepCtx c, float dt, int32_t* bbox_partials) {
    __shared__ int red[6 * (BLOCK / WAVE)];
    const uint32_t i = blockIdx.x * BLOCK + threadIdx.x;
    int mn[3] = {INT_MAX, INT_MAX, INT_MAX}, mx[3] = {INT_MIN, INT_MIN, INT_MIN};
    if (gate_closed(c)) return;
    if (i < c.n) {
        float4 p = c.posm[i];
        const float4 wi = c.w[i];
        p.x += wi.x * dt; p.y += wi.y * dt; p.z += wi.z * dt;
        c.posm[i] = p;
        bool bad = false;
        mn[0] = mx[0] = cell_coord(p.x, c.sc.h, bad);
        mn[1] = mx[1] = cell_coord(p.y, c.sc.h, bad);
        mn[2] = mx[2] = cell_coord(p.z, c.sc.h, bad);
        if (bad) atomicOr(c.flags, 1u);
    }
    block_bbox_store(mn, mx, red, bbox_partials + 6 * blockIdx.x);
}
void launch_update_positions(const StepCtx& c, float dt, int32_t* bbox_partials, int32_t* bbox6, hipStream_t s) {
    if (!c.n) return;
    k_update_positions<<<num_blocks(c.n), BLOCK, 0, s>>>(c, dt, bbox_partials);
    if (bbox6) launch_bbox_final(bbox_partials, num_blocks(c.n), bbox6, s, c.gate);
}

__device__ __forceinline__ void publish_ctl(const SolveCtl* ctl, SolveCtl* pub, uint32_t seq) {
    if (!pub) return;
    typedef uint32_t u32x4 __attribute__((ext_vector_type(4)));
    const u32x4 v = {ctl->done, ctl->iters, __float_as_uint(ctl->err), seq};
    *reinterpret_cast<volatile u32x4*>(pub) = v;
}
constexpr int FINALIZE_THREADS = 1024;
__global__ __launch_bounds__(FINALIZE_THREADS) void k_finalize_error(const float* __restrict__ partials, unsigned nblocks,
                                                                     uint32_t nmodels, const uint32_t* __restrict__ model_counts,
                                                                     SolveCtl* ctl, SolveCtl* pub, const uint32_t* gate, uint32_t* close,
                                                                     uint32_t close_stage, uint32_t skipped) {
    __shared__ float red[FINALIZE_THREADS / WAVE];
    typedef uint32_t u32x4 __attribute__((ext_vector_type(4)));
    if (gate && gate_words_closed(gate[0], gate[1], close_stage)) return;
    const u32x4 c0 = reinterpret_cast<const u32x4*>(ctl)[0], c1 = reinterpret_cast<const u32x4*>(ctl)[1];
    const uint32_t done = c0.x, iters = c0.y + skipped, seq = c0.w + 1u + skipped, min_iter = c1.y, mode = c1.z;
    const float tol = __uint_as_float(c1.x);
    if (done) {
        if (threadIdx.x == 0) { ctl->seq = seq; publish_ctl(ctl, pub, seq); }
        return;
    }
    float best = 0.0f;
    for (uint32_t m = 0; m < nmodels; ++m) {
        const uint32_t cnt = model_counts[m];
        float s = 0.0f;
        for (unsigned b = threadIdx.x; b < nblocks; b += FINALIZE_THREADS) s += partials[(size_t)b * nmodels + m];
        s = block_sum(s, red);
        if (threadIdx.x == 0 && cnt != 0) best = fmaxf(best, s / (float)cnt);
    }
    if (threadIdx.x == 0) {
        const bool ok = best <= tol && iters >= min_iter;
        const u32x4 out = {ok ? 1u : 0u, (mode == 0 && ok) ? iters : iters + 1u, __float_as_uint(best), seq};
        reinterpret_cast<u32x4*>(ctl)[0] = out;
        if (pub) *reinterpret_cast<volatile u32x4*>(pub) = out;
// ... 113 lines not shown
```

### salva_amd/csrc/pairs.h

```cpp
#pragma once
#include <cstdlib>

#include "tile.h"

namespace salva {

struct RecPW { float4 p, w; };
struct RecPK { float4 p; float k; };

__device__ __forceinline__ float rho0_of(const StepCtx& c, uint32_t model) {
    return (c.nmodels == 1) ? c.rho0_single : c.rho0_tab[model];
}

template <uint32_t DS>
__device__ __forceinline__ uint32_t pw_dist(const StepCtx& c, const Tile& t) { return DS ? DS * 16u : (t.stage_cap(c) + t.SB) * 16u; }
template <uint32_t DS>
__device__ __forceinline__ uint32_t pk_dist(const StepCtx& c, const Tile& t) { return DS ? DS * 16u : (t.stage_cap(c) + 2u * t.SB) * 16u; }

__device__ __forceinline__ RecPW load_pw(uint32_t o, uint32_t dist) {
    RecPW r{lds_ld16(o), lds_ld16(o + dist)};
    asm volatile("" ::"v"(r.w.w));
    return r;
}
__device__ __forceinline__ RecPK load_pk(uint32_t o, uint32_t dist) { return RecPK{lds_ld16(o), lds_ld4((o >> 2) + dist)}; }
// ... 120 lines not shown
template <typename K2>
__device__ __forceinline__ void pair_sum_gradient_p2_two(const StepCtx& c, uint32_t gs, uint32_t nqu, const ListRegs& lh, const float4& pi,
                                                         uint32_t dist8, uint32_t na, float ma, float mb, K2&& kij2, float& sx, float& sy, float& sz) {
    f2 ax = {0.0f, 0.0f}, ay = {0.0f, 0.0f}, az = {0.0f, 0.0f};
    const f2 tiny = {1.0e-30f, 1.0e-30f};
    for_each_ff2_indexed<2>(c, gs, nqu, lh, [&](uint32_t o) { return load_p2(o, dist8); }, [&](const RecP2& A, const RecP2& B, uint32_t q) { SALVA_PAIR_MATH
        const f2 dx = {pi.x - A.xy.x, pi.x - B.xy.x}, dy = {pi.y - A.xy.y, pi.y - B.xy.y}, dz = {pi.z - A.zk.x, pi.z - B.zk.x};
        f2 r2 = dz * dz + tiny;
        r2 = dy * dy + r2;
        r2 = dx * dx + r2;
        const f2 g = kernel_gfac2(r2, c.sc);
        const f2 m = {2u * q < na ? ma : mb, 2u * q + 1u < na ? ma : mb};
        const f2 coeff = kij2(A.zk.y, B.zk.y) * (g * m);
        ax += dx * coeff; ay += dy * coeff; az += dz * coeff;
    });
    sx = (ax.x + ax.y) * c.sc.gscale; sy = (ay.x + ay.y) * c.sc.gscale; sz = (az.x + az.y) * c.sc.gscale;
}
template <typename K1>
__device__ __forceinline__ void pair_sum_gradient_exact_p2(const StepCtx& c, uint32_t i, uint32_t gs, const float4& pi, uint32_t dist8,
                                                           float mass, K1&& kij1, float& sx, float& sy, float& sz) {
    float ax = 0.0f, ay = 0.0f, az = 0.0f;
    for_each_ff(c, i, gs, [&](uint32_t s) { SALVA_PAIR_MATH
        const RecP2 A = load_p2(s << 3, dist8);
        const float dx = pi.x - A.xy.x, dy = pi.y - A.xy.y, dz = pi.z - A.zk.x;
        const float coeff = kij1(A.zk.y) * kernel_grad(dx * dx + dy * dy + dz * dz, c.sc);
        ax += dx * coeff; ay += dy * coeff; az += dz * coeff;
    });
    sx = ax * mass; sy = ay * mass; sz = az * mass;
}
template <typename K1>
__device__ __forceinline__ void pair_tail_gradient_p2(const StepCtx& c, uint32_t gs, uint32_t first, uint32_t cnt, const float4& pi, uint32_t dist8,
                                                      K1&& kij1, float& sx, float& sy, float& sz) {
    float ax = 0.0f, ay = 0.0f, az = 0.0f;
    for_each_ff_range(c, gs, first, cnt, [&](uint32_t s) { SALVA_PAIR_MATH
        const RecP2 A = load_p2(s << 3, dist8);
        const float dx = pi.x - A.xy.x, dy = pi.y - A.xy.y, dz = pi.z - A.zk.x;
        const float coeff = kij1(A.zk.y) * kernel_grad(dx * dx + dy * dy + dz * dz, c.sc);
        ax += dx * coeff; ay += dy * coeff; az += dz * coeff;
    });
    sx = ax; sy = ay; sz = az;
}
__device__ __forceinline__ float4 p2_boundary_pos(const Tile& t, uint32_t s, uint32_t dist8) {
    const uint32_t o = (t.S + s) * 8u;
    const lds_v2f xy = lds_ld8(o), zv = lds_ld8(o + dist8);
    return make_float4(xy.x, xy.y, zv.x, zv.y);
}
static inline uint32_t p2_bytes(const TileLds& L, uint32_t ds) {
    const uint32_t n = L.raw_slots();
    const uint32_t dist8 = ds ? ds * 8u : ((n * 8u + 15u) & ~15u);
    return dist8 + n * 8u + 32u;
}

template <typename K2>
__device__ __forceinline__ void pair_sum_gradient(const StepCtx& c, uint32_t gs, uint32_t nqu, const ListRegs& lh, const float4& pi,
                                                  uint32_t dist, K2&& kij2, float& sx, float& sy, float& sz) {
    f2 ax = {0.0f, 0.0f}, ay = {0.0f, 0.0f}, az = {0.0f, 0.0f};
    const f2 tiny = {1.0e-30f, 1.0e-30f};
    for_each_ff2<true, false, true>(c, gs, nqu, lh, [&](uint32_t o) { return load_pk(o, dist); }, [&](const RecPK& A, const RecPK& B) { SALVA_PAIR_MATH
        const f2 dx = {pi.x - A.p.x, pi.x - B.p.x}, dy = {pi.y - A.p.y, pi.y - B.p.y}, dz = {pi.z - A.p.z, pi.z - B.p.z};
        f2 r2 = dz * dz + tiny;
        r2 = dy * dy + r2;
        r2 = dx * dx + r2;
        const f2 g = kernel_gfac2(r2, c.sc);
        const f2 km = kij2(A.k, B.k) * f2{A.p.w, B.p.w};
        const f2 coeff = km * g;
        ax += dx * coeff; ay += dy * coeff; az += dz * coeff;
    });
    sx = (ax.x + ax.y) * c.sc.gscale; sy = (ay.x + ay.y) * c.sc.gscale; sz = (az.x + az.y) * c.sc.gscale;
}
template <typename K1>
__device__ __forceinline__ void pair_sum_gradient_exact(const StepCtx& c, uint32_t i, uint32_t gs, const float4& pi, uint32_t dist,
                                                        K1&& kij1, float& sx, float& sy, float& sz) {
    float ax = 0.0f, ay = 0.0f, az = 0.0f;
    for_each_ff(c, i, gs, [&](uint32_t s) { SALVA_PAIR_MATH
        const RecPK A = load_pk(s << 4, dist);
        const float dx = pi.x - A.p.x, dy = pi.y - A.p.y, dz = pi.z - A.p.z;
        const float coeff = kij1(A.k) * A.p.w * kernel_grad(dx * dx + dy * dy + dz * dz, c.sc);
        ax += dx * coeff; ay += dy * coeff; az += dz * coeff;
    });
    sx = ax; sy = ay; sz = az;
}
__device__ __forceinline__ bool slice_is_near(const StepCtx& c, uint32_t near_word) {
#ifdef SALVA_OTHER_KERNELS
    return (__builtin_amdgcn_readfirstlane((int)near_word) | c.sc.kg) != 0;
#else
    return __builtin_amdgcn_readfirstlane((int)near_word) != 0;
#endif
}
__device__ __forceinline__ float (*carve_errtab(Tile& t))[MAX_MODELS] {
    return reinterpret_cast<float (*)[MAX_MODELS]>(t.carve<float>(TILE_MAX_WAVES * MAX_MODELS));
}

#define SALVA_LAUNCH_FIXED(kernel, DSV, c, L, lds, s, ...)                                                         \
    do {                                                                                                           \
        if ((DSV) == FIXED_DS_SMALL) SALVA_LAUNCH_TILE_3(kernel<FIXED_DS_SMALL>, kernel<FIXED_DS_SMALL>, FIXED_DS_SMALL, kernel<0u>, c, L, lds, s, __VA_ARGS__); \
        else if ((DSV) == FIXED_DS_LARGE) SALVA_LAUNCH_TILE_3(kernel<FIXED_DS_LARGE>, kernel<FIXED_DS_SMALL>, FIXED_DS_SMALL, kernel<0u>, c, L, lds, s, __VA_ARGS__); \
        else SALVA_LAUNCH_TILE_3(kernel<0u>, kernel<FIXED_DS_SMALL>, FIXED_DS_SMALL, kernel<0u>, c, L, lds, s, __VA_ARGS__); \
    } while (0)
static inline uint32_t pick_ds(uint32_t slots_needed, uint32_t level) {
    const uint32_t ds[3] = {FIXED_DS_SMALL, FIXED_DS_LARGE, 0u};
    uint32_t k = slots_needed <= FIXED_DS_SMALL ? 0u : (slots_needed <= FIXED_DS_LARGE ? 1u : 2u);
    k += level;
    return ds[k < 2u ? k : 2u];
}
static inline uint32_t pw_slots(const TileLds& L) { return L.sum_slots(); }
static inline uint32_t pw_bytes(const TileLds& L, uint32_t ds, bool errtab) {
    return (ds ? 2u * ds : 2u * pw_slots(L)) * 16u + (errtab ? TILE_ERR_BYTES : 0u) + 32u;
}
static inline uint32_t pick_ds_p3(uint32_t s, uint32_t level) {
    const uint32_t ds[4] = {P3_DS_THREE, P3_DS_TWO, P3_DS_ONE, 0u};
    uint32_t k = s <= P3_DS_THREE ? 0u : (s <= P3_DS_TWO ? 1u : (s <= P3_DS_ONE ? 2u : 3u));
    k += level;
    return ds[k < 3u ? k : 3u];
}
static inline uint32_t p3_bytes(const TileLds& L, uint32_t ds, uint32_t nmodels, bool with_bv) {
    const uint32_t dist8 = ds ? ds * 8u : ((L.max_halo_fluid * 8u + 15u) & ~15u);
    const uint32_t bb = with_bv ? 32u : 16u;
    const uint32_t by_maxima = ((L.max_halo_fluid * 8u + 15u) & ~15u) + bb * L.max_halo_boundary;
    const uint32_t by_raw = ((L.raw_slots() * 8u + 15u) & ~15u) + (bb - 8u) * L.max_halo_boundary;
    static const uint32_t pad = getenv("SALVA_HIP_P3_PAD") ? (uint32_t)atoi(getenv("SALVA_HIP_P3_PAD")) : 0u;
    return 2u * dist8 + (by_raw < by_maxima ? by_raw : by_maxima) + ((TILE_MAX_WAVES * nmodels * 4u + 15u) & ~15u) + 32u + pad;
}
static inline uint32_t pick_ds_p2(uint32_t n, uint32_t level) {
    const uint32_t ds[4] = {P2_DS_THREE, P3_DS_TWO, P3_DS_ONE, 0u};
    uint32_t k = n <= P2_DS_THREE ? 0u : (n <= P3_DS_TWO ? 1u : (n <= P3_DS_ONE ? 2u : 3u));
    k += level;
    return ds[k < 3u ? k : 3u];
}
#define SALVA_LAUNCH_P3(kernel, DSV, c, L, lds, s, ...)                                                                                          \
    do {                                                                                                                                         \
        if ((DSV) == P3_DS_THREE) SALVA_LAUNCH_TILE_3(kernel<P3_DS_THREE>, kernel<P3_DS_THREE>, P3_DS_THREE, kernel<0u>, c, L, lds, s, __VA_ARGS__); \
        else if ((DSV) == P3_DS_TWO) SALVA_LAUNCH_TILE_3(kernel<P3_DS_TWO>, kernel<P3_DS_THREE>, P3_DS_THREE, kernel<0u>, c, L, lds, s, __VA_ARGS__); \
        else if ((DSV) == P3_DS_ONE) SALVA_LAUNCH_TILE_3(kernel<P3_DS_ONE>, kernel<P3_DS_THREE>, P3_DS_THREE, kernel<0u>, c, L, lds, s, __VA_ARGS__); \
        else SALVA_LAUNCH_TILE_3(kernel<0u>, kernel<P3_DS_THREE>, P3_DS_THREE, kernel<0u>, c, L, lds, s, __VA_ARGS__);                             \
    } while (0)
#define SALVA_LAUNCH_P2(kernel, DSV, c, L, lds, s, ...)                                                                                          \
    do {                                                                                                                                         \
        if ((DSV) == P2_DS_THREE) SALVA_LAUNCH_TILE_3(kernel<P2_DS_THREE>, kernel<P2_DS_THREE>, P2_DS_THREE, kernel<0u>, c, L, lds, s, __VA_ARGS__); \
        else if ((DSV) == P3_DS_TWO) SALVA_LAUNCH_TILE_3(kernel<P3_DS_TWO>, kernel<P2_DS_THREE>, P2_DS_THREE, kernel<0u>, c, L, lds, s, __VA_ARGS__); \
        else if ((DSV) == P3_DS_ONE) SALVA_LAUNCH_TILE_3(kernel<P3_DS_ONE>, kernel<P2_DS_THREE>, P2_DS_THREE, kernel<0u>, c, L, lds, s, __VA_ARGS__); \
        else SALVA_LAUNCH_TILE_3(kernel<0u>, kernel<P2_DS_THREE>, P2_DS_THREE, kernel<0u>, c, L, lds, s, __VA_ARGS__);                             \
    } while (0)
static inline uint32_t pk_slots(const TileLds& L) { return L.sum_slots() + L.max_halo_boundary; }
static inline uint32_t pk_bytes(const TileLds& L, uint32_t ds) {
    return (ds ? ds : pk_slots(L)) * 16u + ((L.max_halo_fluid + 63u) & ~63u) * 4u + 32u;
}


}
```

### salva_amd/csrc/switches.h

```cpp
#pragma once
#include <cstdint>

namespace salva {

struct Switches {
    bool spec_off = true;
    bool spec_tight = false;
    bool defer_off = false;
    bool spec_apply_off = false;
    bool spec_dist_off = false;
    bool overlap_exchange = true;
    bool chain_off = false;
    bool pre_off = false;
    bool no_publish = false;
    bool split_off = false;
    uint32_t split_forced = 0;
    bool classes_off = false, classes_forced = false, light_on = false;
    bool ref_off = false, ref_forced = false;
    bool ref_tight = false;
    bool compact_halo = false;
    bool no_planes = false;
    bool no_fused_div = false;
    bool two_mass_off = false;
    uint32_t max_masses = 2;
    bool fold_off = false;
    uint32_t fold_forced = 0;
    int sort_mode = -1;
    uint32_t ds_level = 0;
    bool trust_cap0 = false;
    uint32_t list_cap0 = 0;
    bool dcs_batch_off = false;
    uint32_t dcsb_cap0 = 0;
    bool tile_trace = false;
    bool dist_trace = false;
#ifdef SALVA_HIP_DIAG
    int sched_mode = 0;
    bool tile_threads_set = false;
    uint32_t tile_threads = 0;
    bool no_pipeline = false;
    uint32_t pipe_waves = 0;
    bool tile_timing = false;
#endif
    static Switches from_env();
};

}
```

### salva_amd/csrc/tile.h

```cpp
#pragma once
#include "common.h"
#include "device_types.h"

namespace salva {

#ifndef SALVA_TX
#define SALVA_TX 4
#endif
constexpr int TX = SALVA_TX, TY = 4, TZ = 4;
constexpr int TCELLS = TX * TY * TZ;
constexpr int HX = TX + 2, HY = TY + 2, HZ = TZ + 2;
constexpr int HCELLS = HX * HY * HZ;
constexpr int TILE_MAX_WAVES = 12;
constexpr int TILE_MAX_THREADS = TILE_MAX_WAVES * WAVE;

__host__ __device__ inline int floor_div(int a, int b) { return (a >= 0) ? a / b : -((-a + b - 1) / b); }

__host__ __device__ inline uint32_t ellq(uint32_t q) { return (q >> 2) * (4u * (uint32_t)WAVE) + (q & 3u); }

constexpr uint32_t TILE_TABLE_BYTES = 4 * (2 * (HCELLS + 1) + 2 * HCELLS) + 16;

struct TileLds {
    uint32_t max_halo_fluid = 0, max_halo_boundary = 0, threads = 4 * WAVE;
    uint32_t max_sum = 0;
// ... 702 lines not shown
        }
    } else {
#pragma unroll
    for (int k = 0; k < LIST_REGS; k += 2) {
        if (FUSED) {
            if ((uint32_t)(k + 1) < nq) {
                const uint32_t a = lr.d[k], b = lr.d[k + 1];
                const auto d0 = load(entry_lo<OFF>(a));
                const auto d1 = load(entry_hi<OFF>(a));
                const auto d2 = load(entry_lo<OFF>(b));
                const auto d3 = load(entry_hi<OFF>(b));
                compute2(d0, d1);
                compute2(d2, d3);
            } else if ((uint32_t)k < nq) {
                const uint32_t a = lr.d[k];
                const auto d0 = load(entry_lo<OFF>(a));
                const auto d1 = load(entry_hi<OFF>(a));
                compute2(d0, d1);
            }
        } else if ((uint32_t)k < nq) {
            const uint32_t a = lr.d[k];
            const bool two = (uint32_t)(k + 1) < nq;
            const uint32_t b = two ? lr.d[k + 1] : a;
            const auto d0 = load(entry_lo<OFF>(a));
            const auto d1 = load(entry_hi<OFF>(a));
            const auto d2 = load(entry_lo<OFF>(b));
            const auto d3 = load(entry_hi<OFF>(b));
            compute2(d0, d1);
            if (two) compute2(d2, d3);
        }
    }
    }
    if (nq > (uint32_t)LIST_REGS) {
        const uint32_t* __restrict__ p = c.nbr_ff + (size_t)gslice * c.cap_ff * WAVE + 4u * (threadIdx.x & (WAVE - 1));
        if (AHEAD) {
            uint32_t nx = p[ellq(LIST_REGS)];
            for (uint32_t q = LIST_REGS; q < nq; ++q) {
                const uint32_t a = nx;
                if (q + 1 < nq) nx = p[ellq(q + 1)];
                const auto d0 = load(entry_lo<OFF>(a));
                const auto d1 = load(entry_hi<OFF>(a));
                compute2(d0, d1);
            }
        } else {
            for (uint32_t q = LIST_REGS; q < nq; ++q) {
                const uint32_t a = p[ellq(q)];
                const auto d0 = load(entry_lo<OFF>(a));
                const auto d1 = load(entry_hi<OFF>(a));
                compute2(d0, d1);
            }
        }
    }
}
template <int OFF, typename L, typename C2>
__device__ __forceinline__ void for_each_ff2_indexed(const StepCtx& c, uint32_t gslice, uint32_t nq, const ListRegs& lr, L&& load, C2&& compute2) {
#pragma unroll
    for (int k = 0; k < LIST_REGS; k += 2) {
        if ((uint32_t)k < nq) {
            const uint32_t a = lr.d[k];
            const bool two = (uint32_t)(k + 1) < nq;
            const uint32_t b = two ? lr.d[k + 1] : a;
            const auto d0 = load(entry_lo<OFF>(a));
            const auto d1 = load(entry_hi<OFF>(a));
            const auto d2 = load(entry_lo<OFF>(b));
            const auto d3 = load(entry_hi<OFF>(b));
            compute2(d0, d1, (uint32_t)k);
            if (two) compute2(d2, d3, (uint32_t)(k + 1));
        }
    }
    if (nq > (uint32_t)LIST_REGS) {
        const uint32_t* __restrict__ p = c.nbr_ff + (size_t)gslice * c.cap_ff * WAVE + 4u * (threadIdx.x & (WAVE - 1));
        uint32_t nx = p[ellq(LIST_REGS)];
        for (uint32_t q = LIST_REGS; q < nq; ++q) {
            const uint32_t a = nx;
            if (q + 1 < nq) nx = p[ellq(q + 1)];
            const auto d0 = load(entry_lo<OFF>(a));
            const auto d1 = load(entry_hi<OFF>(a));
            compute2(d0, d1, q);
        }
    }
}
constexpr int FB_REGS = 8;
struct FbRegs { uint32_t d[FB_REGS]; };
__device__ __forceinline__ FbRegs fb_regs(const StepCtx& c, uint32_t gslice) {
    const uint32_t* __restrict__ p = (c.nb ? c.nbr_fb + (size_t)gslice * c.cap_fb * WAVE : c.nbr_ff + (size_t)gslice * c.cap_ff * WAVE) +
                                     4u * (threadIdx.x & (WAVE - 1));
    static_assert(FB_REGS % 4 == 0, "fetched in 16-byte pieces");
    const uint4* __restrict__ p4 = reinterpret_cast<const uint4*>(p);
    FbRegs r;
#pragma unroll
    for (int k = 0; k < FB_REGS / 4; ++k) {
        const uint4 v = p4[(size_t)k * WAVE];
        r.d[4 * k] = v.x; r.d[4 * k + 1] = v.y; r.d[4 * k + 2] = v.z; r.d[4 * k + 3] = v.w;
    }
    return r;
}
template <typename F>
__device__ __forceinline__ void for_each_fb_regs(const StepCtx& c, uint32_t SB, uint32_t gslice, uint32_t cnt, const FbRegs& fr, F&& f) {
    if (SB == 0 || cnt == 0) return;
    const uint32_t nq = (cnt + 1) >> 1;
#pragma unroll
    for (int k = 0; k < FB_REGS; ++k) {
        if ((uint32_t)k < nq) {
            const uint32_t a = fr.d[k];
            f(a & 0xffffu);
            if (2u * (uint32_t)k + 1u < cnt) f(a >> 16);
        }
    }
    if (nq > (uint32_t)FB_REGS) {
        const uint32_t* __restrict__ p = c.nbr_fb + (size_t)gslice * c.cap_fb * WAVE + 4u * (threadIdx.x & (WAVE - 1));
        for (uint32_t q = FB_REGS; q < nq; ++q) {
            const uint32_t a = p[ellq(q)];
            f(a & 0xffffu);
            if (2u * q + 1u < cnt) f(a >> 16);
        }
    }
}
struct ListOwn { uint32_t cnt; ListRegs lr; };
__device__ __forceinline__ ListOwn list_own(const StepCtx& c, uint32_t i, uint32_t gslice) { return ListOwn{c.nff[i], list_regs(c, gslice)}; }
template <typename L, typename C>
__device__ __forceinline__ void for_each_ff_regs(const StepCtx& c, uint32_t gslice, const ListOwn& o, L&& load, C&& compute) {
    const uint32_t cnt = o.cnt;
#pragma unroll
    for (int k = 0; k < LIST_REGS; ++k) {
        if (2u * (uint32_t)k < cnt) {
            const uint32_t a = o.lr.d[k];
            const auto d0 = load(a & 0xffffu);
            const auto d1 = load(a >> 16);
            compute(d0);
            if (2u * (uint32_t)k + 1u < cnt) compute(d1);
        }
    }
    if (cnt > 2u * (uint32_t)LIST_REGS) {
        const uint32_t* __restrict__ p = c.nbr_ff + (size_t)gslice * c.cap_ff * WAVE + 4u * (threadIdx.x & (WAVE - 1));
        const uint32_t nq = (cnt + 1u) >> 1;
        uint32_t nx = p[ellq(LIST_REGS)];
        for (uint32_t q = LIST_REGS; q < nq; ++q) {
            const uint32_t a = nx;
            if (q + 1 < nq) nx = p[ellq(q + 1)];
            const auto d0 = load(a & 0xffffu);
            const auto d1 = load(a >> 16);
            compute(d0);
            if (2u * q + 1u < cnt) compute(d1);
        }
    }
}
template <typename F>
__device__ __forceinline__ void for_each_ff_regs(const StepCtx& c, uint32_t gslice, const ListOwn& o, F&& f) {
    for_each_ff_regs(c, gslice, o, [](uint32_t s) { return s; }, f);
}
__device__ __forceinline__ uint32_t slice_list_dwords(uint32_t cnt, bool active) {
    return (uint32_t)__builtin_amdgcn_readfirstlane((int)wave_max_u32(active ? ((cnt + 1) >> 1) : 0u));
}
template <typename L, typename C>
__device__ __forceinline__ void for_each_ff(const StepCtx& c, uint32_t i, uint32_t gslice, L&& load, C&& compute) {
    for_each_slot(c.nbr_ff, c.cap_ff, gslice, c.nff[i], load, compute);
}
template <typename F>
__device__ __forceinline__ void for_each_ff(const StepCtx& c, uint32_t i, uint32_t gslice, F&& f) {
    for_each_slot(c.nbr_ff, c.cap_ff, gslice, c.nff[i], [](uint32_t s) { return s; }, f);
}
template <typename F>
__device__ __forceinline__ void for_each_fb(const StepCtx& c, const Tile& t, uint32_t i, uint32_t gslice, F&& f) {
    if (t.SB == 0) return;
    for_each_slot(c.nbr_fb, c.cap_fb, gslice, c.nfb[i], [](uint32_t s) { return s; }, f);
}

__device__ __forceinline__ bool is_ghost(const StepCtx& c, uint32_t i) { return c.gtag && (c.gtag[i] & 0x80000000u); }

constexpr int MAX_MODELS = 32;
struct TileErr {
    float (*tab)[MAX_MODELS];
    __device__ __forceinline__ void init(float (*t)[MAX_MODELS], const StepCtx& c) {
        tab = t;
        const uint32_t lane = threadIdx.x & (WAVE - 1);
        if (lane < c.nmodels) tab[threadIdx.x / WAVE][lane] = 0.0f;
    }
    __device__ __forceinline__ void add(const StepCtx& c, float err, uint32_t mi, bool active) {
        const uint32_t lane = threadIdx.x & (WAVE - 1), wv = threadIdx.x / WAVE;
        if (c.nmodels == 1) {
            const float s = wave_sum(active ? err : 0.0f);
            if (lane == 0) tab[wv][0] += s;
        } else {
            for (uint32_t m = 0; m < c.nmodels; ++m) {
                const float s = wave_sum((active && mi == m) ? err : 0.0f);
                if (lane == 0) tab[wv][m] += s;
            }
        }
    }
    __device__ __forceinline__ void finish(const StepCtx& c, uint32_t tile) {
        __syncthreads();
        if (threadIdx.x < c.nmodels) {
            float s = 0.0f;
            for (int w = 0; w < (int)(blockDim.x / WAVE); ++w) s += tab[w][threadIdx.x];
            c.partials[(size_t)tile * c.nmodels + threadIdx.x] = s;
        }
    }
    static __device__ __forceinline__ void zero(const StepCtx& c, uint32_t tile) {
        if (threadIdx.x < c.nmodels) c.partials[(size_t)tile * c.nmodels + threadIdx.x] = 0.0f;
    }
};

struct TileErrC {
    float* tab;
    uint32_t nm;
    static __device__ __forceinline__ uint32_t bytes(const StepCtx& c) { return (TILE_MAX_WAVES * c.nmodels * 4u + 15u) & ~15u; }
    __device__ __forceinline__ void init(float* t, const StepCtx& c) {
        tab = t; nm = c.nmodels;
        const uint32_t lane = threadIdx.x & (WAVE - 1);
        if (lane < nm) tab[(threadIdx.x / WAVE) * nm + lane] = 0.0f;
    }
    __device__ __forceinline__ void add(const StepCtx& c, float err, uint32_t mi, bool active) {
        const uint32_t lane = threadIdx.x & (WAVE - 1), wv = threadIdx.x / WAVE;
        if (nm == 1) {
            const float s = wave_sum(active ? err : 0.0f);
            if (lane == 0) tab[wv] += s;
        } else {
            for (uint32_t m = 0; m < nm; ++m) {
                const float s = wave_sum((active && mi == m) ? err : 0.0f);
                if (lane == 0) tab[wv * nm + m] += s;
            }
        }
    }
    __device__ __forceinline__ void finish(const StepCtx& c, uint32_t tile) {
        __syncthreads();
        if (threadIdx.x < nm) {
            float s = 0.0f;
            for (int w = 0; w < (int)(blockDim.x / WAVE); ++w) s += tab[(uint32_t)w * nm + threadIdx.x];
            c.partials[(size_t)tile * nm + threadIdx.x] = s;
        }
    }
};

__device__ __forceinline__ void apply_boundary_force(const StepCtx& c, uint32_t jb_sorted, uint32_t bmodel, float fx,
                                                     float fy, float fz) {
    if (c.bforce == nullptr || !c.bwants[bmodel]) return;
    unsigned long long* f = c.bforce_fx + 3ull * c.bperm[jb_sorted];
    atomicAdd(f + 0, (unsigned long long)__float2ll_rn(fx * c.bforce_scale));
    atomicAdd(f + 1, (unsigned long long)__float2ll_rn(fy * c.bforce_scale));
    atomicAdd(f + 2, (unsigned long long)__float2ll_rn(fz * c.bforce_scale));
}
__device__ __forceinline__ uint32_t boundary_sorted_of_slot(const StepCtx& c, const Tile& t, uint32_t slot) {
    return c.bhalo_src[t.hboff + slot];
}

struct ContactRow {
    const uint32_t* p;
    uint64_t hoff;
// ... 25 lines not shown
```

### salva_amd/csrc/world.hip

```cpp
#include "world.h"
#include "bbox.h"

#include <algorithm>
#include <cmath>
#include <cstring>
#include <limits>

#include <mutex>
#include <unordered_map>

namespace salva {

void raise_tile_lds_limit(const void* kernel, uint32_t bytes) {
    if (bytes > 160u * 1024u)
        throw HipError(SALVA_HIP_E_CAPACITY, "a tile's halo does not fit the 160 KiB LDS (particles are compressed far beyond rest density)");
    static std::mutex mu;
    static std::unordered_map<const void*, uint32_t> granted;
    std::lock_guard<std::mutex> lock(mu);
    uint32_t& g = granted[kernel];
    if (bytes <= g) return;
    const uint32_t want = std::min<uint32_t>(160u * 1024u, std::max<uint32_t>(bytes + bytes / 4, 64u * 1024u));
    SALVA_HIP_CHECK(hipFuncSetAttribute(kernel, hipFuncAttributeMaxDynamicSharedMemorySize, (int)want));
    g = want;
}

int bits_for(uint64_t ncells) {
    int b = 1;
    while (b < 32 && ((uint64_t)1 << b) < ncells) ++b;
    return b;
}

Switches Switches::from_env() {
    Switches s;
    auto on = [](const char* name) { return getenv(name) != nullptr; };
    s.spec_dist_off = on("SALVA_HIP_NO_SPEC_DIST");
    s.overlap_exchange = !on("SALVA_HIP_NO_OVERLAP");
    s.spec_off = !on("SALVA_HIP_SPECULATE") || on("SALVA_HIP_NO_SPECULATION");
    s.spec_tight = on("SALVA_HIP_SPEC_TIGHT");
    s.defer_off = on("SALVA_HIP_NO_DEFER_LISTS");
    s.spec_apply_off = on("SALVA_HIP_NO_SPEC_APPLY");
    s.chain_off = on("SALVA_HIP_NO_CHAIN");
    s.pre_off = on("SALVA_HIP_NO_PREGRID");
    s.no_publish = on("SALVA_HIP_NO_PUBLISH");
    s.split_off = on("SALVA_HIP_NO_SPLIT");
    s.classes_off = on("SALVA_HIP_NO_CLASSES");
    s.classes_forced = on("SALVA_HIP_CLASSES");
    s.light_on = on("SALVA_HIP_LIGHT");
    s.ref_off = on("SALVA_HIP_FULL_HALO");
    s.ref_forced = on("SALVA_HIP_REF_HALO");
    s.ref_tight = on("SALVA_HIP_REF_TIGHT");
    s.compact_halo = on("SALVA_HIP_COMPACT_HALO");
    if (const char* e = getenv("SALVA_HIP_SPLIT_S")) s.split_forced = (uint32_t)std::max(atoi(e), 1);
    s.no_planes = on("SALVA_HIP_NO_PLANES");
    s.two_mass_off = on("SALVA_HIP_NO_TWO_MASS");
    if (const char* e = getenv("SALVA_HIP_MAX_MASSES")) s.max_masses = (uint32_t)std::min(std::max(atoi(e), 2), 4);
    s.fold_off = on("SALVA_HIP_NO_FOLD");
    if (const char* e = getenv("SALVA_HIP_FOLD_CELLS")) {
        const long v = atol(e);
        if (v >= 8 && v <= (1 << 20) && (v & (v - 1)) == 0) s.fold_forced = (uint32_t)v;
    }
    s.tile_trace = on("SALVA_HIP_TILE_TRACE");
    s.dist_trace = on("SALVA_HIP_DIST_TRACE");
    s.no_fused_div = on("SALVA_HIP_NO_FUSED_DIV");
    s.dcs_batch_off = on("SALVA_HIP_NO_DCS_BATCH");
    if (const char* e = getenv("SALVA_HIP_DCSB_CAP0")) s.dcsb_cap0 = (uint32_t)std::max(atoi(e), 1);
    if (const char* e = getenv("SALVA_HIP_RADIX_SORT")) s.sort_mode = atoi(e) != 0 ? 1 : 0;
    if (const char* e = getenv("SALVA_HIP_DS_LEVEL")) s.ds_level = (uint32_t)std::max(0, atoi(e));
    if (const char* e = getenv("SALVA_HIP_LIST_CAP0")) { s.list_cap0 = std::max<uint32_t>(LIST_REGS, ((uint32_t)atoi(e) + 3u) & ~3u); s.trust_cap0 = true; }
#ifdef SALVA_HIP_DIAG
    if (const char* e = getenv("SALVA_HIP_SCHED")) s.sched_mode = atoi(e);
    if (const char* e = getenv("SALVA_HIP_TILE_THREADS")) { s.tile_threads = (uint32_t)atoi(e); s.tile_threads_set = true; }
    s.no_pipeline = on("SALVA_HIP_NO_PIPELINE");
    if (const char* e = getenv("SALVA_HIP_PIPE_WAVES")) s.pipe_waves = std::min<uint32_t>(std::max(atoi(e), 1), PIPE_MAX_WAVES);
    s.tile_timing = on("SALVA_HIP_TILE_TIMING");
#endif
    return s;
}

World::World(const SalvaHipParams& p) : prm(p) {
    if (!(p.particle_radius > 0.0f) || !(p.smoothing_factor > 0.0f))
        throw HipError(SALVA_HIP_E_INVALID, "particle_radius and smoothing_factor must be positive");
    if (p.solver != SALVA_HIP_SOLVER_DFSPH && p.solver != SALVA_HIP_SOLVER_IISPH)
        throw HipError(SALVA_HIP_E_INVALID, "unknown solver kind");
    int ndev = 0;
    hipError_t e = hipGetDeviceCount(&ndev);
    if (e != hipSuccess || ndev == 0)
        throw HipError(SALVA_HIP_E_HIP, "no HIP device available: libsalva_hip has no CPU fallback");
    if (p.device < 0 || p.device >= ndev) throw HipError(SALVA_HIP_E_INVALID, "device ordinal out of range");
    use_device();
    const float h = p.particle_radius * p.smoothing_factor * 2.0f;
    sc = make_sph_consts(h);
    if (p.kernel_density < 0 || p.kernel_density > SALVA_HIP_KERNEL_VISCOSITY || p.kernel_gradient < 0 || p.kernel_gradient > SALVA_HIP_KERNEL_VISCOSITY)
        throw HipError(SALVA_HIP_E_INVALID, "unknown kernel kind");
    sc.kd = p.kernel_density;
    sc.kg = p.kernel_gradient;
    SALVA_HIP_CHECK(hipStreamCreateWithFlags(&stream, hipStreamNonBlocking));
    SALVA_HIP_CHECK(hipStreamCreateWithFlags(&stream2, hipStreamNonBlocking));
    SALVA_HIP_CHECK(hipEventCreateWithFlags(&ev_pre_refresh, hipEventDisableTiming));
    SALVA_HIP_CHECK(hipEventCreateWithFlags(&ev_interior, hipEventDisableTiming));
    SALVA_HIP_CHECK(hipEventCreateWithFlags(&ev_spec_eval, hipEventDisableTiming));
    SALVA_HIP_CHECK(hipEventCreateWithFlags(&ev_spec_apply, hipEventDisableTiming));
    lds.ds_level = sw.ds_level;
    if (sw.trust_cap0) cap_ff = sw.list_cap0;
    {
        int cus = 0;
        if (hipDeviceGetAttribute(&cus, hipDeviceAttributeMultiprocessorCount, p.device) == hipSuccess && cus > 0) num_cus = cus;
    }
    SALVA_HIP_CHECK(hipHostMalloc((void**)&h_rb, sizeof(Readback), hipHostMallocDefault));
    memset(h_rb, 0, sizeof(Readback));
    SALVA_HIP_CHECK(hipHostMalloc((void**)&h_ctl, 2 * NUM_SOLVES * sizeof(SolveCtl), hipHostMallocDefault));
    memset(h_ctl, 0, 2 * NUM_SOLVES * sizeof(SolveCtl));
    SALVA_HIP_CHECK(hipHostMalloc((void**)&h_pub, NUM_SOLVES * sizeof(SolveCtl), hipHostMallocMapped | hipHostMallocCoherent));
    memset(h_pub, 0, NUM_SOLVES * sizeof(SolveCtl));
    SALVA_HIP_CHECK(hipHostMalloc((void**)&h_hostpub, sizeof(HostPub), hipHostMallocMapped | hipHostMallocCoherent));
    memset(h_hostpub, 0, sizeof(HostPub));
    d_ctl.ensure(NUM_SOLVES);
    d_rb.ensure(1);
    d_flags.p = &d_rb.p->flags;
    SALVA_HIP_CHECK(hipMemset(d_rb.p, 0, sizeof(Readback)));
    {
        mass_slots.ensure(2 * MASS_SLOTS);
        SALVA_HIP_CHECK(hipMemset(mass_slots.p, 0, 2 * MASS_SLOTS * sizeof(uint32_t)));
    }
    d_counters.ensure(4);
    for (auto& e2 : ev) SALVA_HIP_CHECK(hipEventCreate(&e2));
    for (auto& e2 : evc) SALVA_HIP_CHECK(hipEventCreate(&e2));
    SALVA_HIP_CHECK(hipEventCreateWithFlags(&ev_sync, hipEventDisableTiming));
}

World::~World() {
    (void)hipSetDevice(prm.device);
    if (stream) { (void)hipStreamSynchronize(stream); (void)hipStreamDestroy(stream); }
    if (stream2) { (void)hipStreamSynchronize(stream2); (void)hipStreamDestroy(stream2); }
    if (dl_stream) { (void)hipStreamSynchronize(dl_stream); (void)hipStreamDestroy(dl_stream); }
    if (ev_dl_ready) (void)hipEventDestroy(ev_dl_ready);
    if (ev_dl_done) (void)hipEventDestroy(ev_dl_done);
    for (float* p : h_dl) if (p) (void)hipHostFree(p);
    for (hipEvent_t e : dist_ev) if (e) (void)hipEventDestroy(e);
    if (ev_pre_refresh) (void)hipEventDestroy(ev_pre_refresh);
    if (ev_interior) (void)hipEventDestroy(ev_interior);
    if (ev_spec_eval) (void)hipEventDestroy(ev_spec_eval);
    if (ev_spec_apply) (void)hipEventDestroy(ev_spec_apply);
    if (h_rb) (void)hipHostFree(h_rb);
    if (h_ctl) (void)hipHostFree(h_ctl);
    if (h_pub) (void)hipHostFree(h_pub);
    if (h_hostpub) (void)hipHostFree(h_hostpub);
// ... 47 lines not shown
    for (uint32_t a = 0; a < fluids.size(); ++a) {
        r0[a] = fluids[a].density0;
        counts[a] = (uint32_t)fluids[a].n;
        for (uint32_t b = 0; b < fluids.size(); ++b)
            ff[a * nm + b] = (a == b) || groups_test(fluids[a].memberships, fluids[a].filter, fluids[b].memberships, fluids[b].filter);
        for (uint32_t b = 0; b < bounds.size(); ++b)
            fb[a * nbm + b] = groups_test(fluids[a].memberships, fluids[a].filter, bounds[b].memberships, bounds[b].filter);
    }
    for (uint32_t a = 0; a < bounds.size(); ++a) {
        bw[a] = bounds[a].wants_forces ? 1 : 0;
        any_wants_forces |= bounds[a].wants_forces;
        for (uint32_t b = 0; b < bounds.size(); ++b)
            bb[a * nbm + b] = (a == b) || groups_test(bounds[a].memberships, bounds[a].filter, bounds[b].memberships, bounds[b].filter);
    }
    rho0_tab.ensure(nm); model_counts.ensure(nm); ff_ok.ensure(nm * nm); fb_ok.ensure(nm * nbm); bb_ok.ensure(nbm * nbm); bwants.ensure(nbm);
    SALVA_HIP_CHECK(hipMemcpyAsync(rho0_tab.p, r0.data(), nm * sizeof(float), hipMemcpyHostToDevice, stream));
    if (comm && dist_started && global_counts.size() == nm) counts = global_counts;
    SALVA_HIP_CHECK(hipMemcpyAsync(model_counts.p, counts.data(), nm * sizeof(uint32_t), hipMemcpyHostToDevice, stream));
    SALVA_HIP_CHECK(hipMemcpyAsync(ff_ok.p, ff.data(), ff.size(), hipMemcpyHostToDevice, stream));
    SALVA_HIP_CHECK(hipMemcpyAsync(fb_ok.p, fb.data(), fb.size(), hipMemcpyHostToDevice, stream));
    SALVA_HIP_CHECK(hipMemcpyAsync(bb_ok.p, bb.data(), bb.size(), hipMemcpyHostToDevice, stream));
    SALVA_HIP_CHECK(hipMemcpyAsync(bwants.p, bw.data(), bw.size(), hipMemcpyHostToDevice, stream));
    SALVA_HIP_CHECK(hipStreamSynchronize(stream));
    tables_dirty = false;
    b_dirty = true;
}

float World::bforce_scale() const {
    const float r = prm.particle_radius;
    return std::exp2f(36.0f - std::ceil(std::log2(1000.0f * r * r * r)));
}

StepCtx World::make_ctx() {
    StepCtx c{};
    if (any_wants_forces && bforce_fx_n != nb) {
        bforce_fx.ensure(3 * (size_t)std::max<uint32_t>(nb, 1u), stream, false, 1.2f);
        SALVA_HIP_CHECK(hipMemsetAsync(bforce_fx.p, 0, 3 * (size_t)std::max<uint32_t>(nb, 1u) * sizeof(unsigned long long), stream));
        bforce_fx_n = nb;
    }
    c.sc = sc;
    {
        uint32_t lg = 1u;
        while (lg < 7u && (16u << lg) <= pass.nlaunch) ++lg;
        c.xcd = lg;
    }
    c.n = n;
    c.posm = posm[cur].p; c.vel = vel[cur].p; c.dv = dv[cur].p; c.acc = acc.p; c.w = w.p; c.normal = normal.p;
    c.model = model[cur].p; c.perm = perm[cur].p; c.gtag = comm ? gtag[cur].p : nullptr;
    c.rho = rho.p; c.alpha = alpha.p; c.kappa = kappa.p; c.kappa2 = kappa2.p; c.rho_star = rho_star.p; c.aii = aii.p;
    c.dii = dii.p; c.dijpj = dijpj.p; c.iisph_q = iisph_q.p; c.iisph_pr = iisph_pr.p; c.posmr = posmr.p;
    c.nff = nff.p; c.nfb = nfb.p;
    c.nbr_ff = nbr_ff.p; c.nbr_fb = nbr_fb.p; c.cap_ff = cap_ff; c.cap_fb = cap_fb;
    c.slice_near = slice_near.p;
    c.tile_off = G().tile_off.p; c.halo_src = halo_src.p; c.bhalo_src = bhalo_src.p;
    c.halo_stride = halo_stride; c.bhalo_stride = bhalo_stride;
    c.ntiles = (uint32_t)gf.ntiles();
    c.split_s = pass.split_s_cur;
    c.slot_order = (pass.class_ntiny || pass.class_nlight) ? slot_order.p : nullptr; c.slot_base = 0u; c.ntiny = pass.class_ntiny; c.nlight = pass.class_nlight;
    c.tile_ids = G().tile_ids.p; c.tile_rank = G().tile_rank.p; c.nlaunch = pass.nlaunch; c.slot_desc = G().slot_desc.p; c.slot_info = slot_info.p;
    c.spec = pass.spec_mode ? 1u : 0u; c.halo_cap = pass.halo_cap; c.bhalo_cap = pass.bhalo_cap; c.nslices_cap = pass.nslices_cap;
    c.halo_len = pass.halo_len; c.bhalo_len = pass.bhalo_len;
    c.gf = gf.device(G().cell_start_f.p);
    c.stale_keys = has_dynamic_sampling() ? G().keys[1].p : nullptr;
    c.nb = nb;
    c.bposv = bposv.p; c.bvel = bvel.p; c.bperm = bperm.p;
    c.bforce = any_wants_forces ? bforce.p : nullptr;
    c.bforce_fx = any_wants_forces ? bforce_fx.p : nullptr;
    c.bforce_scale = bforce_scale();
    c.bwants = bwants.p;
    c.gb = gb.device(cell_start_b.p);
    c.nmodels = num_models();
    c.nbmodels = (uint32_t)std::max<size_t>(bounds.size(), 1);
    c.mass_uniform = mass_uniform;
    c.two_mass = pass.two_mass ? 1u : 0u;
    c.nmass = pass.two_mass ? pass.nmass : 0u; c.cmask = pass.mass_cmask;
    for (int k = 0; k < 4; ++k) c.class_mass[k] = pass.mass_classes[k];
    c.tile_mass_bits = pass.two_mass ? tile_mass_bits.p : nullptr;
    c.tile_massb_bits = pass.two_mass ? tile_massb_bits.p : nullptr;
    c.tile_masscd_bits = (pass.two_mass && pass.nmass > 2u) ? tile_masscd_bits.p : nullptr;
    c.nffb = pass.two_mass ? nffb.p : nullptr;
    c.nffc = (pass.two_mass && pass.nmass > 2u) ? nffc.p : nullptr;
    c.bvel_zero = 1u;
    for (const BoundarySlot& b : bounds) if (b.n && (!b.vel_zero || b.sampling || b.dyn)) c.bvel_zero = 0u;
    c.rho0_tab = rho0_tab.p; c.rho0_single = fluids.empty() ? 1000.0f : fluids[0].density0; c.ff_ok = ff_ok.p; c.fb_ok = fb_ok.p; c.bb_ok = bb_ok.p;
    c.partials = partials.p;
    c.spec_k = -1; c.spec_ring = spec_ring.p; c.spec_pub = nullptr; c.model_counts = model_counts.p; c.w2 = w2.p;
    c.flags = d_flags.p;
    c.min_neighbors_for_divergence = 20;
    c.phase = 0;
    c.ghost_lo_cx = (comm && comm->has_lo()) ? slab_lo - 1 : INT32_MIN;
    c.ghost_hi_cx = (comm && comm->has_hi()) ? slab_hi + 1 : INT32_MAX;
    return c;
}

void dims_from_bbox(const int32_t* bb, GridDims& g, const FoldRule* fold) {
    static const int T[3] = {TX, TY, TZ};
    int64_t cells[3];
    for (int a = 0; a < 3; ++a) {
        if (bb[a] > bb[3 + a]) throw HipError(SALVA_HIP_E_CAPACITY, "empty cell bounding box");
        const int64_t extent = (int64_t)bb[3 + a] - (int64_t)bb[a] + 1;
        if (extent > (1 << 30)) throw HipError(SALVA_HIP_E_CAPACITY, "cell bounding box too large");
        g.o[a] = bb[a];
        g.nt[a] = (int)((extent + T[a] - 1) / T[a]);
        g.mask[a] = 0xffffffffu;
        cells[a] = (int64_t)g.nt[a] * T[a];
    }
    if (fold && (double)cells[0] * (double)cells[1] * (double)cells[2] > fold->budget) {
        for (;;) {
            if ((double)cells[0] * (double)cells[1] * (double)cells[2] <= fold->target) break;
            int best = -1;
            int64_t best_p = 0;
            for (int a = 0; a < 3; ++a) {
                int64_t p = 1;
                while (p * 2 < cells[a]) p *= 2;
                if (!fold->axis[a] || p < (int64_t)fold->min_period[a] || p >= cells[a]) continue;
                if (best < 0 || cells[a] > cells[best]) { best = a; best_p = p; }
            }
            if (best < 0) break;
            cells[best] = best_p;
            g.nt[best] = (int)(best_p / T[best]);
            g.mask[best] = (uint32_t)best_p - 1u;
        }
    }
    const double nc = (double)cells[0] * (double)cells[1] * (double)cells[2];
    if (nc >= 4.0e9) throw HipError(SALVA_HIP_E_CAPACITY, "dense cell table would exceed 2^32 cells; particles are too spread out");
    static const double budget_gib = [] {
        const char* e = getenv("SALVA_HIP_CELL_TABLE_GIB");
        const double v = e ? atof(e) : 8.0;
        return v > 0.0 ? v : 8.0;
    }();
    const double gib = (nc * 4.0 + nc / TCELLS * 8.0) / (1024.0 * 1024.0 * 1024.0);
    if (gib > budget_gib) {
        char msg[512];
        snprintf(msg, sizeof msg,
                 "the cell table over the particles' bounding box (%d x %d x %d tiles of %dx%dx%d cells) would take %.1f GiB, over the "
                 "%.1f GiB budget: particles are too spread out for the dense grid — delete strays (salva_hip_particles_intersecting_aabb "
                 "+ salva_hip_delete_particles) or raise SALVA_HIP_CELL_TABLE_GIB",
                 g.nt[0], g.nt[1], g.nt[2], TX, TY, TZ, gib, budget_gib);
        throw HipError(SALVA_HIP_E_CAPACITY, msg);
    }
}

void World::build_boundary_grid() {
    if (!b_dirty) return;
    ncontacts_bb = 0;
    if (nb == 0) { b_dirty = false; return; }
    bbox_partials.ensure(6 * std::max<size_t>(bbox_blocks(nb), 1024));
    launch_bbox(bst_pos.p, nb, sc.h, bbox_partials.p, d_rb.p->bbbox, d_flags.p, stream);
    SALVA_HIP_CHECK(hipMemcpyAsync(h_rb->bbbox, d_rb.p->bbbox, sizeof(int32_t) * 6, hipMemcpyDeviceToHost, stream));
    SALVA_HIP_CHECK(hipStreamSynchronize(stream));
    dims_from_bbox(h_rb->bbbox, gb);
    const size_t nc = gb.ncells();
    bkeys[0].ensure(nb); bkeys[1].ensure(nb); bidx[0].ensure(nb); bidx[1].ensure(nb);
    bposv.ensure(nb); bvel.ensure(nb); bperm.ensure(nb); cell_start_b.ensure(nc + 1);
    TileGrid gv = gb.device(nullptr);
    launch_cell_keys(bst_pos.p, nb, sc.h, gv, bkeys[0].p, bidx[0].p, d_flags.p, nullptr, nullptr, nullptr, stream);
    const int end_bit = bits_for(nc);
    const size_t tb = sort_pairs_temp_bytes(nb, end_bit);
    ensure_cub_temp(tb);
    sort_pairs(cub_temp.p, tb, bkeys[0].p, bkeys[1].p, bidx[0].p, bidx[1].p, nb, end_bit, stream);
    launch_reorder_boundary(nb, bidx[1].p, bst_pos.p, bst_vel.p, bposv.p, bvel.p, bperm.p, stream);
    launch_cell_start(bkeys[1].p, nb, (uint32_t)nc, cell_start_b.p, stream);
    StepCtx c = make_ctx();
    SALVA_HIP_CHECK(hipMemsetAsync(d_counters.p + 2, 0, sizeof(unsigned long long), stream));
    launch_boundary_volumes(c, d_counters.p + 2, stream);
    SALVA_HIP_CHECK(hipMemcpyAsync(&h_rb->ncontacts_bb, d_counters.p + 2, sizeof(uint64_t), hipMemcpyDeviceToHost, stream));
// ... 182 lines not shown
```

### salva_amd/csrc/world_io.hip

```cpp
#include "world.h"

#include <algorithm>
#include <cstring>

namespace salva {

__global__ void k_unpack_xyz(uint32_t n, const float4* __restrict__ src, float* __restrict__ dst) {
    const uint32_t i = blockIdx.x * BLOCK + threadIdx.x;
    if (i >= n) return;
    const float4 s = src[i];
    dst[3 * i] = s.x; dst[3 * i + 1] = s.y; dst[3 * i + 2] = s.z;
}
__global__ void k_unpack_w(uint32_t n, const float4* __restrict__ src, float* __restrict__ dst) {
    const uint32_t i = blockIdx.x * BLOCK + threadIdx.x;
    if (i < n) dst[i] = src[i].w;
}

void World::download_f32(const float* src, uint64_t count, float* out) {
    SALVA_HIP_CHECK(hipMemcpyAsync(out, src, count * sizeof(float), hipMemcpyDeviceToHost, stream));
    SALVA_HIP_CHECK(hipStreamSynchronize(stream));
}
void World::download_xyz(const float4* src, uint64_t count, float* out) {
    scratch_f.ensure(3 * count, stream, false, 1.1f);
    k_unpack_xyz<<<nblk(count), BLOCK, 0, stream>>>((uint32_t)count, src, scratch_f.p);
// ... 23 lines not shown
    const float4 v = src[s];
    dst[3 * (size_t)h] = v.x; dst[3 * (size_t)h + 1] = v.y; dst[3 * (size_t)h + 2] = v.z;
}
static bool host_pointer_is_pinned(const void* p) {
    hipPointerAttribute_t a{};
    const hipError_t e = hipPointerGetAttributes(&a, p);
    if (e != hipSuccess) { (void)hipGetLastError(); return false; }
    return a.type == hipMemoryTypeHost;
}
void World::get_fluid_async(uint32_t slot, float* pos, float* vel_out) {
    use_device();
    const SlotSpan sp = fluid_span(slot);
    if (comm && dist_started) throw HipError(SALVA_HIP_E_INVALID, "host-order fluid arrays are not maintained in a multi-GPU run: use salva_hip_get_owned");
    wait_download();
    const uint64_t nn = sp.n, off = sp.off;
    if (nn == 0 || (!pos && !vel_out)) return;
    if (!dl_stream) {
        SALVA_HIP_CHECK(hipStreamCreateWithFlags(&dl_stream, hipStreamNonBlocking));
        SALVA_HIP_CHECK(hipEventCreateWithFlags(&ev_dl_ready, hipEventDisableTiming));
        SALVA_HIP_CHECK(hipEventCreateWithFlags(&ev_dl_done, hipEventDisableTiming));
    }
    const size_t bytes = 3 * nn * sizeof(float);
    float* dsts[2] = {pos, vel_out};
    const float4* sorted_src[2] = {posm[cur].p, vel[cur].p};
    const float4* staged_src[2] = {st_pos.p + off, st_vel.p + off};
    const bool from_sorted = sorted_valid && !staging_current;
    for (int a = 0; a < 2; ++a) {
        if (!dsts[a]) continue;
        dl_dev[a].ensure(3 * nn, stream, false, 1.1f);
        if (from_sorted) k_scatter_xyz<<<nblk(n), BLOCK, 0, stream>>>(n, perm[cur].p, (uint32_t)off, (uint32_t)nn, sorted_src[a], dl_dev[a].p);
        else k_unpack_xyz<<<nblk(nn), BLOCK, 0, stream>>>((uint32_t)nn, staged_src[a], dl_dev[a].p);
    }
    SALVA_HIP_CHECK(hipGetLastError());
    SALVA_HIP_CHECK(hipEventRecord(ev_dl_ready, stream));
    SALVA_HIP_CHECK(hipStreamWaitEvent(dl_stream, ev_dl_ready, 0));
    dl = PendingDownload{};
    dl.bytes = bytes;
    for (int a = 0; a < 2; ++a) {
        if (!dsts[a]) continue;
        dl.dst[a] = dsts[a];
        dl.staged[a] = !host_pointer_is_pinned(dsts[a]);
        float* target = dsts[a];
        if (dl.staged[a]) {
            if (h_dl_cap[a] < bytes) {
                if (h_dl[a]) SALVA_HIP_CHECK(hipHostFree(h_dl[a]));
                h_dl[a] = nullptr; h_dl_cap[a] = 0;
                const size_t cap = bytes + bytes / 8;
                SALVA_HIP_CHECK(hipHostMalloc((void**)&h_dl[a], cap, hipHostMallocDefault));
                h_dl_cap[a] = cap;
            }
            target = h_dl[a];
        }
        SALVA_HIP_CHECK(hipMemcpyAsync(target, dl_dev[a].p, bytes, hipMemcpyDeviceToHost, dl_stream));
    }
    SALVA_HIP_CHECK(hipEventRecord(ev_dl_done, dl_stream));
    dl.active = true;
}
void World::wait_download() {
    if (!dl.active) return;
    use_device();
    dl.active = false;
    SALVA_HIP_CHECK(hipEventSynchronize(ev_dl_done));
    for (int a = 0; a < 2; ++a)
        if (dl.dst[a] && dl.staged[a]) memcpy(dl.dst[a], h_dl[a], dl.bytes);
}

void World::get_fluid_field(uint32_t slot, int field, float* out) {
    use_device();
    const SlotSpan sp = fluid_span(slot);
    if (!out) throw HipError(SALVA_HIP_E_INVALID, "null output");
    if (comm && dist_started) throw HipError(SALVA_HIP_E_INVALID, "per-fluid host-order access is not available in a multi-GPU run: use salva_hip_get_owned");
    const uint64_t nn = sp.n, off = sp.off;
    if (nn == 0) return;
    enum Part { XYZ, W, F32, U32_AS_F32 };
    struct Source { const void* array; Part part; bool staged; };
    Source src{nullptr, F32, false};
    switch (field) {
        case SALVA_HIP_FIELD_VELOCITY_CHANGE: src = {st_dv.p, XYZ, true}; break;
        case SALVA_HIP_FIELD_PRESSURE: src = {st_dv.p, W, true}; break;
        case SALVA_HIP_FIELD_VOLUME: src = {st_pos.p, W, true}; break;
        case SALVA_HIP_FIELD_ACCELERATION: src = {st_acc.p, XYZ, true}; break;
        case SALVA_HIP_FIELD_DENSITY: src = {rho.p, F32, false}; break;
        case SALVA_HIP_FIELD_ALPHA: src = {alpha.p, F32, false}; break;
        case SALVA_HIP_FIELD_NUM_FLUID_CONTACTS: src = {nff.p, U32_AS_F32, false}; break;
        case SALVA_HIP_FIELD_NUM_BOUNDARY_CONTACTS: src = {nfb.p, U32_AS_F32, false}; break;
        default: break;
    }
    scratch_f.ensure(std::max<size_t>(3 * nn, n), stream, false, 1.1f);
    if (src.staged) {
        if (field == SALVA_HIP_FIELD_ACCELERATION) {
            if (!acc_user) { memset(out, 0, 3 * nn * sizeof(float)); return; }
        } else {
            ensure_staging_current();
        }
        const float4* rows = static_cast<const float4*>(src.array) + off;
        if (src.part == XYZ) download_xyz(rows, nn, out);
        else download_w(rows, nn, out);
        return;
    }
    if (!sorted_valid || !have_last_ctx)
        throw HipError(SALVA_HIP_E_INVALID, "solver scratch fields are only available right after a step");
    if (field == SALVA_HIP_FIELD_NUM_BOUNDARY_CONTACTS && nb == 0) { memset(out, 0, nn * sizeof(float)); return; }
    if (!src.array) throw HipError(SALVA_HIP_E_INVALID, "unknown field");
    if (src.part == F32) launch_unsort_f32(n, perm[cur].p, static_cast<const float*>(src.array), scratch_f.p, stream);
    else launch_unsort_u32_as_f32(n, perm[cur].p, static_cast<const uint32_t*>(src.array), scratch_f.p, stream);
    download_f32(scratch_f.p + off, nn, out);
}

void World::set_fluid_field(uint32_t slot, int field, const float* data) {
    use_device();
    const SlotSpan sp = fluid_span(slot);
    if (!data) throw HipError(SALVA_HIP_E_INVALID, "null data");
    if (field != SALVA_HIP_FIELD_VELOCITY_CHANGE && field != SALVA_HIP_FIELD_PRESSURE)
        throw HipError(SALVA_HIP_E_INVALID, "only velocity_changes and pressures can be set");
    if (sp.n == 0) return;
    ensure_staging_current();
    if (field == SALVA_HIP_FIELD_VELOCITY_CHANGE) upload_xyz(data, st_dv.p + sp.off, sp.n, true);
    else upload_w(data, st_dv.p + sp.off, sp.n);
    order_invalidated(false);
}

void World::get_force_stats(uint32_t slot, uint32_t force, int32_t* iters, float* err) {
    if (slot >= fluids.size() || force >= fluids[slot].forces.size()) throw HipError(SALVA_HIP_E_INVALID, "fluid slot / force index out of range");
    const FluidSlot& f = fluids[slot];
    if (iters) *iters = force < f.force_iters.size() ? (int32_t)f.force_iters[force] : 0;
    if (err) *err = force < f.force_errs.size() ? f.force_errs[force] : 0.0f;
}

void World::get_boundary(uint32_t slot, float* volumes, float* forces) {
    use_device();
    const SlotSpan sp = boundary_span(slot);
    if (sp.n == 0) return;
    if (volumes) {
        upload_tables();
        build_boundary_grid();
        scratch_f4.ensure(nb);
        scratch_f.ensure(nb, stream, false, 1.1f);
        launch_unsort_f4(nb, bperm.p, bposv.p, scratch_f4.p, stream);
        download_w(scratch_f4.p + sp.off, sp.n, volumes);
    }
    if (forces) download_xyz(bforce.p + sp.off, sp.n, forces);
}

void World::get_boundary_particles(uint32_t slot, float* positions, float* velocities) {
    use_device();
    const SlotSpan sp = boundary_span(slot);
    if (sp.n == 0) return;
    if (positions) download_xyz(bst_pos.p + sp.off, sp.n, positions);
    if (velocities) download_xyz(bst_vel.p + sp.off, sp.n, velocities);
}

template <typename Launch>
uint64_t World::export_contacts(uint64_t rows, const uint32_t* d_counts, bool with_moff, uint64_t* offsets, uint32_t* j_model, uint32_t* j,
                                uint64_t capacity, Launch&& launch) {
    std::vector<uint32_t> cnt(rows, 0);
    if (d_counts && rows) {
        SALVA_HIP_CHECK(hipMemcpyAsync(cnt.data(), d_counts, rows * sizeof(uint32_t), hipMemcpyDeviceToHost, stream));
        SALVA_HIP_CHECK(hipStreamSynchronize(stream));
    }
    std::vector<uint64_t> offs(rows + 1, 0);
    for (uint64_t k = 0; k < rows; ++k) offs[k + 1] = offs[k] + cnt[k];
    const uint64_t total = offs[rows];
    if (offsets) memcpy(offsets, offs.data(), (rows + 1) * sizeof(uint64_t));
    if (!j_model || !j || capacity < total || total == 0) return total;
    std::vector<uint32_t> moff, boff(std::max<size_t>(bounds.size(), 1), 0);
    if (with_moff) {
// ... 188 lines not shown
```

### salva_amd/world.py

```python
from __future__ import annotations

import ctypes as C
from dataclasses import dataclass, field
from typing import List, Optional, Sequence

import numpy as np

from . import _lib as L

F32 = np.float32


def _fp(a: Optional[np.ndarray]):
    return a.ctypes.data_as(C.POINTER(C.c_float)) if a is not None else None


def _as_vec3(a, n=None) -> np.ndarray:
    a = np.ascontiguousarray(a, dtype=F32).reshape(-1, 3)
    if n is not None and len(a) != n:
        raise ValueError(f"expected {n} 3-vectors, got {len(a)}")
    return a


@dataclass(frozen=True)
# ... 1195 lines not shown
            except BaseException as e:
                errors.append(e)
                return 1

        cb = L.COUPLING_CALLBACK(callback)
        L.check(self._L.salva_hip_set_coupling_callback(self._h, cb, None))
        try:
            st = self.step(dt, gravity)
        except Exception:
            if errors:
                raise errors[0]
            raise
        finally:
            self._L.salva_hip_set_coupling_callback(self._h, L.COUPLING_CALLBACK(), None)
            if hasattr(coupling, "raise_pending"):
                coupling.raise_pending()
        return st

    def set_domain(self, comm, cell_lo: int, cell_hi: int, gid_offset: int = 0):
        self.sync_to_device()
        L.check(self._L.salva_hip_set_domain(self._h, comm._h, int(cell_lo), int(cell_hi), int(gid_offset)))
        self._comm = comm

    def dist_timing(self):
        out = (C.c_double * 4)()
        L.check(self._L.salva_hip_get_dist_timing(self._h, out))
        return {"refresh_ms": out[0], "refreshes": int(out[1]), "test_ms": out[2], "tests": int(out[3])}

    def delete_owned(self, gids) -> int:
        g = np.ascontiguousarray(gids, np.uint32).ravel()
        m = int(self._L.salva_hip_delete_owned(self._h, len(g), g.ctypes.data_as(C.POINTER(C.c_uint32))))
        if m < 0:
            L.check(m)
        return m

    def add_owned(self, fluid, positions, velocities=None):
        pos = np.ascontiguousarray(positions, np.float32).reshape(-1, 3)
        vel = None if velocities is None else np.ascontiguousarray(velocities, np.float32).reshape(-1, 3)
        L.check(self._L.salva_hip_add_particles(self._h, fluid._slot, len(pos), _fp(pos) if len(pos) else None, _fp(vel) if vel is not None and len(pos) else None))

    def rebalance(self):
        lo, hi = C.c_int32(0), C.c_int32(0)
        L.check(self._L.salva_hip_rebalance(self._h, C.byref(lo), C.byref(hi)))
        return int(lo.value), int(hi.value)

    def owned(self):
        u32p = C.POINTER(C.c_uint32)
        cap = max(int(self.last_stats.nparticles) + 1024, 1024)
        while True:
            gid = np.zeros(cap, np.uint32)
            slot = np.zeros(cap, np.uint32)
            pos = np.zeros((cap, 3), F32)
            vel = np.zeros((cap, 3), F32)
            m = int(self._L.salva_hip_get_owned(self._h, cap, gid.ctypes.data_as(u32p), _fp(pos), _fp(vel),
                                                slot.ctypes.data_as(u32p)))
            if m < 0:
                L.check(m)
            if m <= cap:
                break
            cap = m
        o = np.argsort(gid[:m], kind="stable")
        return gid[:m][o], pos[:m][o], vel[:m][o], slot[:m][o]

    def fluid_field(self, f: Fluid, field: int) -> np.ndarray:
        n = f.num_particles()
        vec = field in (L.FIELD_VELOCITY_CHANGE, L.FIELD_ACCELERATION)
        out = np.zeros((n, 3) if vec else n, F32)
        if n:
            L.check(self._L.salva_hip_get_fluid_field(self._h, f._slot, field, _fp(out)))
        return out

    def densities(self, f: Fluid) -> np.ndarray:
        return self.fluid_field(f, L.FIELD_DENSITY)

    def alphas(self, f: Fluid) -> np.ndarray:
        return self.fluid_field(f, L.FIELD_ALPHA)

    def velocity_changes(self, f: Fluid) -> np.ndarray:
        return self.fluid_field(f, L.FIELD_VELOCITY_CHANGE)

    def pressures(self, f: Fluid) -> np.ndarray:
        return self.fluid_field(f, L.FIELD_PRESSURE)

    def contact_counts(self, f: Fluid, boundary_contacts: bool = False) -> np.ndarray:
        fld = L.FIELD_NUM_BOUNDARY_CONTACTS if boundary_contacts else L.FIELD_NUM_FLUID_CONTACTS
        return self.fluid_field(f, fld).astype(np.uint32)

    def fluid_contacts(self, f: Fluid, boundary_contacts: bool = False):
        n = f.num_particles()
        offsets = np.zeros(n + 1, np.uint64)
        u64p, u32p = C.POINTER(C.c_uint64), C.POINTER(C.c_uint32)
        total = int(self._L.salva_hip_get_fluid_contacts(self._h, f._slot, int(boundary_contacts), offsets.ctypes.data_as(u64p), None, None, 0))
        if total < 0:
            L.check(total)
        jm, j = np.zeros(total, np.uint32), np.zeros(total, np.uint32)
        if total:
            got = int(self._L.salva_hip_get_fluid_contacts(self._h, f._slot, int(boundary_contacts), offsets.ctypes.data_as(u64p),
                                                           jm.ctypes.data_as(u32p), j.ctypes.data_as(u32p), total))
            if got < 0:
                L.check(got)
        return offsets, jm, j

    def particles_intersecting_aabb(self, mins, maxs):
        self.sync_to_device(apply_removal=False)
        lo = (C.c_float * 3)(*[float(x) for x in mins])
        hi = (C.c_float * 3)(*[float(x) for x in maxs])
        u32p = C.POINTER(C.c_uint32)
        cap = 1024
        while True:
            k, s, i = np.zeros(cap, np.uint32), np.zeros(cap, np.uint32), np.zeros(cap, np.uint32)
            total = int(self._L.salva_hip_particles_intersecting_aabb(self._h, lo, hi, cap, k.ctypes.data_as(u32p),
                                                                       s.ctypes.data_as(u32p), i.ctypes.data_as(u32p)))
            if total < 0:
                L.check(total)
            if total <= cap:
                break
            cap = total
        out = []
        for q in range(total):
            owner = self._boundaries._items[int(s[q])] if k[q] else self._fluids._items[int(s[q])]
            out.append(("boundary" if k[q] else "fluid", owner, int(i[q])))
        return out

    def particles_intersecting_shape(self, translation, rotation, shape):
        self.sync_to_device(apply_removal=False)
        from .coupling import make_shape
        from .sampling import Compound, Mesh

        if isinstance(shape, Compound):
            handle = shape.handle(self)
            call = lambda *a: self._L.salva_hip_particles_intersecting_compound(self._h, t, q, handle, *a)
        elif isinstance(shape, Mesh):
            handle = shape.handle(self)
            call = lambda *a: self._L.salva_hip_particles_intersecting_mesh(self._h, t, q, handle, *a)
        else:
            sh = make_shape(shape)
            call = lambda *a: self._L.salva_hip_particles_intersecting_shape(self._h, t, q, C.byref(sh), *a)
        t = (C.c_float * 3)(*[float(x) for x in translation])
        q = (C.c_float * 4)(*[float(x) for x in rotation])
        u32p = C.POINTER(C.c_uint32)
        cap = 1024
        while True:
            k, s, i = np.zeros(cap, np.uint32), np.zeros(cap, np.uint32), np.zeros(cap, np.uint32)
            total = int(call(cap, k.ctypes.data_as(u32p), s.ctypes.data_as(u32p), i.ctypes.data_as(u32p)))
            if total < 0:
                L.check(total)
            if total <= cap:
                break
            cap = total
        out = []
        for j in range(total):
            owner = self._boundaries._items[int(s[j])] if k[j] else self._fluids._items[int(s[j])]
            out.append(("boundary" if k[j] else "fluid", owner, int(i[j])))
        return out

    def particles_intersecting_host_shape(self, compute_aabb, distance_to_point):
        self.sync_to_device(apply_removal=False)
        err = []

        def aabb_cb(_user, mins, maxs):
            try:
                lo, hi = compute_aabb()
                for a in range(3):
                    mins[a], maxs[a] = float(lo[a]), float(hi[a])
            except BaseException as e:
                err.append(e)
# ... 68 lines not shown
```

Baseline: 410.6 million.

## Encode per-slice wall-list size in near word and prefetch boundary lists into registers

The density kernels now pack into the per-slice near word the wave-maximum number of boundary-neighbour dwords, alongside the existing near bit. The pressure and divergence kernels read that count uniformly and use a new for_each_wall path. It prefetches the first boundary neighbour-list dwords into registers before the per-particle tail loads, then runs a software-pipelined loop that issues four boundary loads before computing them. Slices without wall contacts skip the boundary loop entirely. A kappa field getter is also exposed, and an env switch turns the path off; in exchange the loop adds register pressure and depends on the packed count staying in sync.

Measured after the change: 410.6 million (median of 3 runs). No clear change (-0.0%).

```diff
diff --git a/bindings/rust/salva3d-hip/src/ffi.rs b/bindings/rust/salva3d-hip/src/ffi.rs
--- a/bindings/rust/salva3d-hip/src/ffi.rs
+++ b/bindings/rust/salva3d-hip/src/ffi.rs
@@ -46,6 +46,7 @@
 pub const SALVA_HIP_FIELD_PRESSURE: i32 = 5;
 pub const SALVA_HIP_FIELD_VOLUME: i32 = 6;
 pub const SALVA_HIP_FIELD_ACCELERATION: i32 = 7;
+pub const SALVA_HIP_FIELD_KAPPA: i32 = 8;
 
 pub const SALVA_HIP_SHAPE_BALL: i32 = 1;
 pub const SALVA_HIP_SHAPE_CUBOID: i32 = 2;
diff --git a/include/salva_hip.h b/include/salva_hip.h
--- a/include/salva_hip.h
+++ b/include/salva_hip.h
@@ -122,7 +122,8 @@
     SALVA_HIP_FIELD_VELOCITY_CHANGE = 4,
     SALVA_HIP_FIELD_PRESSURE = 5,
     SALVA_HIP_FIELD_VOLUME = 6,
-    SALVA_HIP_FIELD_ACCELERATION = 7
+    SALVA_HIP_FIELD_ACCELERATION = 7,
+    SALVA_HIP_FIELD_KAPPA = 8
 };
 
 void salva_hip_default_params(SalvaHipParams* out);
diff --git a/salva_amd/_lib.py b/salva_amd/_lib.py
--- a/salva_amd/_lib.py
+++ b/salva_amd/_lib.py
@@ -17,7 +17,7 @@
 DEVICE_NEEDS_FF, DEVICE_NEEDS_FB, DEVICE_NEEDS_KERNEL = 1, 2, 4
 DIRTY_POSITIONS, DIRTY_VELOCITIES, DIRTY_VOLUMES, DIRTY_ACCELERATIONS, DIRTY_ALL = 1, 2, 4, 8, 15
 (FIELD_DENSITY, FIELD_ALPHA, FIELD_NUM_FLUID_CONTACTS, FIELD_NUM_BOUNDARY_CONTACTS, FIELD_VELOCITY_CHANGE,
- FIELD_PRESSURE, FIELD_VOLUME, FIELD_ACCELERATION) = range(8)
+ FIELD_PRESSURE, FIELD_VOLUME, FIELD_ACCELERATION, FIELD_KAPPA) = range(9)
 
 EXPORTED_SYMBOLS = [
     "salva_hip_default_params", "salva_hip_create", "salva_hip_destroy", "salva_hip_h", "salva_hip_set_fluid",
diff --git a/salva_amd/csrc/device_types.h b/salva_amd/csrc/device_types.h
--- a/salva_amd/csrc/device_types.h
+++ b/salva_amd/csrc/device_types.h
@@ -127,6 +127,7 @@
     uint64_t cmask;
     float class_mass[4];
     uint32_t bvel_zero;
+    uint32_t wall_regs;
     const uint8_t* ff_ok;
     const uint8_t* fb_ok;
     const uint8_t* bb_ok;
diff --git a/salva_amd/csrc/dfsph.hip b/salva_amd/csrc/dfsph.hip
--- a/salva_amd/csrc/dfsph.hip
+++ b/salva_amd/csrc/dfsph.hip
@@ -114,7 +114,9 @@
             }
             c.posmr[i] = make_float4(pi.x, pi.y, pi.z, pi.w / rho);
         }
-        if ((threadIdx.x & (WAVE - 1)) == 0) c.slice_near[gs] = any_near ? 1u : 0u;
+        asm volatile("" ::: "memory");
+        const uint32_t wallq = slice_list_dwords((active && c.nb) ? c.nfb[i] : 0u, active);
+        if ((threadIdx.x & (WAVE - 1)) == 0) c.slice_near[gs] = slice_wall_word(any_near, wallq);
     });
 }
 void launch_density_alpha(const StepCtx& c, const TileLds& L, float iisph_dt, hipStream_t s) {
@@ -223,7 +225,7 @@
             }
         }
         float err = 0.0f;
-        uint32_t mi = 0;
+        uint32_t mi = 0, cntb = 0;
         if (active) {
             mi = c.model[i];
             const float rho0 = rho0_of(c, mi);
@@ -245,12 +247,13 @@
             c.rho[i] = rho;
             c.alpha[i] = alpha;
             c.posmr[i] = make_float4(pi.x, pi.y, pi.z, c.posm[i].w / rho);
-            const uint32_t cntb = c.nb ? c.nfb[i] : 0u;
+            cntb = c.nb ? c.nfb[i] : 0u;
             div = (o.cnt + cntb >= c.min_neighbors_for_divergence) ? fmaxf(div, 0.0f) : 0.0f;
             c.kappa[i] = div * alpha;
             err = div / rho0;
         }
-        if ((threadIdx.x & (WAVE - 1)) == 0) c.slice_near[gs] = any_near ? 1u : 0u;
+        const uint32_t wallq = slice_list_dwords(cntb, active);
+        if ((threadIdx.x & (WAVE - 1)) == 0) c.slice_near[gs] = slice_wall_word(any_near, wallq);
         E.add(c, err, mi, active && !is_ghost(c, i));
     });
     E.finish(c, t.slot);
@@ -342,6 +345,7 @@
     t.for_own_pre(own0, load_own, [&](const Own& o, uint32_t i, uint32_t gs, bool active) {
         const uint32_t nqu = slice_list_dwords(o.cnt, active);
         const bool near = slice_is_near(c, o.near);
+        const uint32_t wq = slice_wall_dwords(o.near);
         float err = 0.0f;
         uint32_t mi = 0;
         if (active) {
@@ -352,7 +356,7 @@
                 const float4 pi = o.pi, wi = o.wi;
                 div += near ? pair_sum_velocity_divergence_exact(c, i, gs, pi, wi, dist)
                             : pair_sum_velocity_divergence(c, gs, nqu, o.lh, pi, wi, dist);
-                for_each_fb(c, t, i, gs, [&](uint32_t s) { SALVA_PAIR_MATH
+                for_each_wall(c, t, i, gs, wq, [] {}, [&](uint32_t s) { SALVA_PAIR_MATH
                     const float4 pj = Bp[s];
                     const float dx = pi.x - pj.x, dy = pi.y - pj.y, dz = pi.z - pj.z;
                     const float g = kernel_grad(dx * dx + dy * dy + dz * dz, c.sc);
@@ -401,6 +405,7 @@
     t.for_own_pre(own0, load_own, [&](const Own& o, uint32_t i, uint32_t gs, bool active) {
         const uint32_t nqu = slice_list_dwords(o.cnt, active);
         const bool near = slice_is_near(c, o.near);
+        const uint32_t wq = slice_wall_dwords(o.near);
         float err = 0.0f;
         uint32_t mi = 0;
         if (active) {
@@ -422,7 +427,7 @@
                     if (l2) div += (t.massc - t.massb) * pair_tail_velocity_divergence_p3(c, gs, o.cnt - l3 - l2, o.cnt - l3, pi, wi, dist8);
                     if (l3) div += (t.massd - t.massb) * pair_tail_velocity_divergence_p3(c, gs, o.cnt - l3, o.cnt, pi, wi, dist8);
                 }
-                for_each_fb(c, t, i, gs, [&](uint32_t s) { SALVA_PAIR_MATH
+                for_each_wall(c, t, i, gs, wq, [] {}, [&](uint32_t s) { SALVA_PAIR_MATH
                     const float4 pj = Bp[s];
                     const float dx = pi.x - pj.x, dy = pi.y - pj.y, dz = pi.z - pj.z;
                     const float g = kernel_grad(dx * dx + dy * dy + dz * dz, c.sc);
@@ -486,6 +491,7 @@
     t.for_own_pre(own0, load_own, [&](const Own& o, uint32_t i, uint32_t gs, bool active) {
         const uint32_t nqu = slice_list_dwords(o.cnt, active);
         const bool near = slice_is_near(c, o.near);
+        const uint32_t wq = slice_wall_dwords(o.near);
         if (!active) return;
         const float4 pi = o.pi;
         const uint32_t mi = __float_as_uint(o.wi.w);
@@ -496,7 +502,7 @@
         if (near) pair_sum_gradient_exact(c, i, gs, pi, dist, [&](float kj) { return ki + kj; }, sx, sy, sz);
         else pair_sum_gradient(c, gs, nqu, o.lh, pi, dist, [&](float ka, float kb) { return f2{ki + ka, ki + kb}; }, sx, sy, sz);
         d.x -= sx; d.y -= sy; d.z -= sz;
-        for_each_fb(c, t, i, gs, [&](uint32_t s) { SALVA_PAIR_MATH
+        for_each_wall(c, t, i, gs, wq, [] {}, [&](uint32_t s) { SALVA_PAIR_MATH
             const float4 pj = Bp[s];
             const float dx = pi.x - pj.x, dy = pi.y - pj.y, dz = pi.z - pj.z;
             const float g = kernel_grad(dx * dx + dy * dy + dz * dz, c.sc);
@@ -544,6 +550,7 @@
     t.for_own_pre(own0, load_own, [&](const Own& o, uint32_t i, uint32_t gs, bool active) {
         const uint32_t nqu = slice_list_dwords(o.cnt, active);
         const bool near = slice_is_near(c, o.near);
+        const uint32_t wq = slice_wall_dwords(o.near);
         if (!active) return;
         const float4 pi = make_float4(o.px, o.py, o.pz, 0.0f);
         const float ki = o.ki;
@@ -574,11 +581,13 @@
                 sx += dm * bx; sy += dm * by; sz += dm * bz;
             }
         }
-        float4 d = win[i];
-        const uint32_t mi = __float_as_uint(d.w);
-        const float rho0 = rho0_of(c, mi);
-        d.x -= sx; d.y -= sy; d.z -= sz;
-        for_each_fb(c, t, i, gs, [&](uint32_t s) { SALVA_PAIR_MATH
+        float4 d;
+        float rho0;
+        for_each_wall(c, t, i, gs, wq, [&] {
+            d = win[i];
+            rho0 = rho0_of(c, __float_as_uint(d.w));
+            d.x -= sx; d.y -= sy; d.z -= sz;
+        }, [&](uint32_t s) { SALVA_PAIR_MATH
             const float4 pj = p2_boundary_pos(t, s, dist8);
             const float dx = pi.x - pj.x, dy = pi.y - pj.y, dz = pi.z - pj.z;
             const float g = kernel_grad(dx * dx + dy * dy + dz * dz, c.sc);
@@ -678,6 +687,7 @@
     t.for_own_pre(own0, load_own, [&](const Own& o, uint32_t i, uint32_t gs, bool active) {
         const uint32_t nqu = slice_list_dwords(o.cnt, active);
         const bool near = slice_is_near(c, o.near);
+        const uint32_t wq = slice_wall_dwords(o.near);
         float err = 0.0f;
         uint32_t mi = 0;
         if (active) {
@@ -686,7 +696,7 @@
             const float4 pi = o.pi, wi = o.wi;
             float delta = near ? pair_sum_velocity_divergence_exact(c, i, gs, pi, wi, dist)
                                : pair_sum_velocity_divergence(c, gs, nqu, o.lh, pi, wi, dist);
-            for_each_fb(c, t, i, gs, [&](uint32_t s) { SALVA_PAIR_MATH
+            for_each_wall(c, t, i, gs, wq, [] {}, [&](uint32_t s) { SALVA_PAIR_MATH
                 const float4 pj = Bp[s];
                 const float4 vj = Bv[s];
                 const float dx = pi.x - pj.x, dy = pi.y - pj.y, dz = pi.z - pj.z;
@@ -739,6 +749,7 @@
     t.for_own_pre(own0, load_own, [&](const Own& o, uint32_t i, uint32_t gs, bool active) {
         const uint32_t nqu = slice_list_dwords(o.cnt, active);
         const bool near = slice_is_near(c, o.near);
+        const uint32_t wq = slice_wall_dwords(o.near);
         float err = 0.0f;
         uint32_t mi = 0;
         if (active) {
@@ -757,9 +768,11 @@
                 if (l2) delta += (t.massc - t.massb) * pair_tail_velocity_divergence_p3(c, gs, o.cnt - l3 - l2, o.cnt - l3, pi, wi, dist8);
                 if (l3) delta += (t.massd - t.massb) * pair_tail_velocity_divergence_p3(c, gs, o.cnt - l3, o.cnt, pi, wi, dist8);
             }
-            mi = POST ? c.model[i] : o.mi;
-            const float rho0 = rho0_of(c, mi);
-            for_each_fb(c, t, i, gs, [&](uint32_t s) { SALVA_PAIR_MATH
+            float rho0;
+            for_each_wall(c, t, i, gs, wq, [&] {
+                mi = POST ? c.model[i] : o.mi;
+                rho0 = rho0_of(c, mi);
+            }, [&](uint32_t s) { SALVA_PAIR_MATH
                 const float4 pj = Bp[s];
                 const float4 vj = c.bvel_zero ? make_float4(0.0f, 0.0f, 0.0f, 0.0f) : Bv[s];
                 const float dx = pi.x - pj.x, dy = pi.y - pj.y, dz = pi.z - pj.z;
@@ -816,6 +829,7 @@
     t.for_own_pre(own0, load_own, [&](const Own& o, uint32_t i, uint32_t gs, bool active) {
         const uint32_t nqu = slice_list_dwords(o.cnt, active);
         const bool near = slice_is_near(c, o.near);
+        const uint32_t wq = slice_wall_dwords(o.near);
         if (!active) return;
         const float4 pi = o.pi;
         const uint32_t mi = o.mi;
@@ -827,8 +841,8 @@
         if (near) pair_sum_gradient_exact(c, i, gs, pi, dist, [&](float kj) { return kip + fmaxf(kj, 0.0f); }, sx, sy, sz);
         else pair_sum_gradient(c, gs, nqu, o.lh, pi, dist, [&](float ka, float kb) { return f2{kip + fmaxf(ka, 0.0f), kip + fmaxf(kb, 0.0f)}; }, sx, sy, sz);
         d.x -= sx * inv_dt; d.y -= sy * inv_dt; d.z -= sz * inv_dt;
-        if (ki > 0.0f) {
-            for_each_fb(c, t, i, gs, [&](uint32_t s) { SALVA_PAIR_MATH
+        {
+            for_each_wall(c, t, i, gs, wq, [] {}, [&](uint32_t s) { SALVA_PAIR_MATH
                 const float4 pj = Bp[s];
                 const float dx = pi.x - pj.x, dy = pi.y - pj.y, dz = pi.z - pj.z;
                 const float g = kernel_grad(dx * dx + dy * dy + dz * dz, c.sc);
@@ -839,7 +853,7 @@
                     const float fs = inv_dt * pi.w;
                     apply_boundary_force(c, boundary_sorted_of_slot(c, t, s), __float_as_uint(Bv[s].w), ex * fs, ey * fs, ez * fs);
                 }
-            });
+            }, ki > 0.0f);
         }
         c.dv[i] = d;
         const float4 v = o.v;
@@ -867,6 +881,7 @@
     t.for_own_pre(own0, load_own, [&](const Own& o, uint32_t i, uint32_t gs, bool active) {
         const uint32_t nqu = slice_list_dwords(o.cnt, active);
         const bool near = slice_is_near(c, o.near);
+        const uint32_t wq = slice_wall_dwords(o.near);
         if (!active) return;
         const float4 pi = make_float4(o.px, o.py, o.pz, 0.0f);
         const float ki = o.ki;
@@ -899,12 +914,16 @@
                 sx += dm * bx; sy += dm * by; sz += dm * bz;
             }
         }
-        const uint32_t mi = c.model[i];
-        const float rho0 = rho0_of(c, mi);
-        float4 d = c.dv[i];
-        d.x -= sx * inv_dt; d.y -= sy * inv_dt; d.z -= sz * inv_dt;
-        if (ki > 0.0f) {
-            for_each_fb(c, t, i, gs, [&](uint32_t s) { SALVA_PAIR_MATH
+        uint32_t mi;
+        float rho0;
+        float4 d;
+        {
+            for_each_wall(c, t, i, gs, wq, [&] {
+                mi = c.model[i];
+                rho0 = rho0_of(c, mi);
+                d = c.dv[i];
+                d.x -= sx * inv_dt; d.y -= sy * inv_dt; d.z -= sz * inv_dt;
+            }, [&](uint32_t s) { SALVA_PAIR_MATH
                 const float4 pj = p2_boundary_pos(t, s, dist8);
                 const float dx = pi.x - pj.x, dy = pi.y - pj.y, dz = pi.z - pj.z;
                 const float g = kernel_grad(dx * dx + dy * dy + dz * dz, c.sc);
@@ -916,7 +935,7 @@
                     const uint32_t jb = boundary_sorted_of_slot(c, t, s);
                     apply_boundary_force(c, jb, __float_as_uint(c.bvel[jb].w), ex * fs, ey * fs, ez * fs);
                 }
-            });
+            }, ki > 0.0f);
         }
         c.dv[i] = d;
         const float4 v = c.vel[i];
diff --git a/salva_amd/csrc/pairs.h b/salva_amd/csrc/pairs.h
--- a/salva_amd/csrc/pairs.h
+++ b/salva_amd/csrc/pairs.h
@@ -226,9 +226,9 @@
 }
 __device__ __forceinline__ bool slice_is_near(const StepCtx& c, uint32_t near_word) {
 #ifdef SALVA_OTHER_KERNELS
-    return (__builtin_amdgcn_readfirstlane((int)near_word) | c.sc.kg) != 0;
+    return ((__builtin_amdgcn_readfirstlane((int)near_word) & 1) | c.sc.kg) != 0;
 #else
-    return __builtin_amdgcn_readfirstlane((int)near_word) != 0;
+    return (__builtin_amdgcn_readfirstlane((int)near_word) & 1) != 0;
 #endif
 }
 __device__ __forceinline__ float (*carve_errtab(Tile& t))[MAX_MODELS] {
diff --git a/salva_amd/csrc/switches.h b/salva_amd/csrc/switches.h
--- a/salva_amd/csrc/switches.h
+++ b/salva_amd/csrc/switches.h
@@ -21,6 +21,7 @@
     bool compact_halo = false;
     bool no_planes = false;
     bool no_fused_div = false;
+    bool no_wall_regs = false;
     bool two_mass_off = false;
     uint32_t max_masses = 2;
     bool fold_off = false;
diff --git a/salva_amd/csrc/tile.h b/salva_amd/csrc/tile.h
--- a/salva_amd/csrc/tile.h
+++ b/salva_amd/csrc/tile.h
@@ -808,9 +808,7 @@
 }
 constexpr int FB_REGS = 8;
 struct FbRegs { uint32_t d[FB_REGS]; };
-__device__ __forceinline__ FbRegs fb_regs(const StepCtx& c, uint32_t gslice) {
-    const uint32_t* __restrict__ p = (c.nb ? c.nbr_fb + (size_t)gslice * c.cap_fb * WAVE : c.nbr_ff + (size_t)gslice * c.cap_ff * WAVE) +
-                                     4u * (threadIdx.x & (WAVE - 1));
+__device__ __forceinline__ FbRegs fb_regs_at(const uint32_t* __restrict__ p) {
     static_assert(FB_REGS % 4 == 0, "fetched in 16-byte pieces");
     const uint4* __restrict__ p4 = reinterpret_cast<const uint4*>(p);
     FbRegs r;
@@ -820,6 +818,10 @@
         r.d[4 * k] = v.x; r.d[4 * k + 1] = v.y; r.d[4 * k + 2] = v.z; r.d[4 * k + 3] = v.w;
     }
     return r;
+}
+__device__ __forceinline__ FbRegs fb_regs(const StepCtx& c, uint32_t gslice) {
+    return fb_regs_at((c.nb ? c.nbr_fb + (size_t)gslice * c.cap_fb * WAVE : c.nbr_ff + (size_t)gslice * c.cap_ff * WAVE) +
+                      4u * (threadIdx.x & (WAVE - 1)));
 }
 template <typename F>
 __device__ __forceinline__ void for_each_fb_regs(const StepCtx& c, uint32_t SB, uint32_t gslice, uint32_t cnt, const FbRegs& fr, F&& f) {
@@ -840,6 +842,39 @@
             f(a & 0xffffu);
             if (2u * q + 1u < cnt) f(a >> 16);
         }
+    }
+}
+template <typename L, typename C>
+__device__ __forceinline__ void for_each_slot_head(const uint32_t* __restrict__ p, uint32_t cnt, FbRegs fr, L&& load, C&& compute) {
+    if (cnt == 0) return;
+    const uint32_t nq = (cnt + 1) >> 1;
+    uint32_t q = 0;
+    uint32_t n0 = fr.d[0], n1 = fr.d[1];
+#pragma clang loop unroll(disable)
+    for (; q + 2 <= nq; q += 2) {
+        const uint32_t a = n0, b = n1;
+#pragma unroll
+        for (int k = 0; k + 2 < FB_REGS; ++k) fr.d[k] = fr.d[k + 2];
+        n0 = fr.d[0]; n1 = fr.d[1];
+        if (q + 2 >= (uint32_t)FB_REGS) {
+            if (q + 2 < nq) n0 = p[ellq(q + 2)];
+            if (q + 3 < nq) n1 = p[ellq(q + 3)];
+        }
+        const auto d0 = load(a & 0xffffu);
+        const auto d1 = load(a >> 16);
+        const auto d2 = load(b & 0xffffu);
+        const auto d3 = load(b >> 16);
+        compute(d0);
+        compute(d1);
+        compute(d2);
+        if (2 * q + 3 < cnt) compute(d3);
+    }
+    if (q < nq) {
+        const uint32_t a = n0;
+        const auto d0 = load(a & 0xffffu);
+        const auto d1 = load(a >> 16);
+        compute(d0);
+        if (2 * q + 1 < cnt) compute(d1);
     }
 }
 struct ListOwn { uint32_t cnt; ListRegs lr; };
@@ -890,6 +925,25 @@
 __device__ __forceinline__ void for_each_fb(const StepCtx& c, const Tile& t, uint32_t i, uint32_t gslice, F&& f) {
     if (t.SB == 0) return;
     for_each_slot(c.nbr_fb, c.cap_fb, gslice, c.nfb[i], [](uint32_t s) { return s; }, f);
+}
+__device__ __forceinline__ uint32_t slice_wall_word(bool any_near, uint32_t wall_dwords) { return (any_near ? 1u : 0u) | (wall_dwords << 1); }
+__device__ __forceinline__ uint32_t slice_wall_dwords(uint32_t wall_word) {
+    return (uint32_t)__builtin_amdgcn_readfirstlane((int)wall_word) >> 1;
+}
+template <typename Post, typename F>
+__device__ __forceinline__ void for_each_wall(const StepCtx& c, const Tile& t, uint32_t i, uint32_t gslice, uint32_t wq, Post&& post, F&& f,
+                                              bool lane_on = true) {
+    const bool regs = c.wall_regs != 0u && wq != 0u && t.SB != 0u;
+    if (regs) {
+        const uint32_t cnt = c.nfb[i];
+        const uint32_t* __restrict__ p = c.nbr_fb + (size_t)gslice * c.cap_fb * WAVE + 4u * (threadIdx.x & (WAVE - 1));
+        const FbRegs fr = fb_regs_at(p);
+        post();
+        for_each_slot_head(p, lane_on ? cnt : 0u, fr, [](uint32_t sl) { return sl; }, f);
+    } else {
+        post();
+        if (c.wall_regs == 0u && lane_on) for_each_fb(c, t, i, gslice, f);
+    }
 }
 
 __device__ __forceinline__ bool is_ghost(const StepCtx& c, uint32_t i) { return c.gtag && (c.gtag[i] & 0x80000000u); }
diff --git a/salva_amd/csrc/world.hip b/salva_amd/csrc/world.hip
--- a/salva_amd/csrc/world.hip
+++ b/salva_amd/csrc/world.hip
@@ -62,6 +62,7 @@
     s.tile_trace = on("SALVA_HIP_TILE_TRACE");
     s.dist_trace = on("SALVA_HIP_DIST_TRACE");
     s.no_fused_div = on("SALVA_HIP_NO_FUSED_DIV");
+    s.no_wall_regs = on("SALVA_HIP_NO_WALL_REGS");
     s.dcs_batch_off = on("SALVA_HIP_NO_DCS_BATCH");
     if (const char* e = getenv("SALVA_HIP_DCSB_CAP0")) s.dcsb_cap0 = (uint32_t)std::max(atoi(e), 1);
     if (const char* e = getenv("SALVA_HIP_RADIX_SORT")) s.sort_mode = atoi(e) != 0 ? 1 : 0;
@@ -275,6 +276,7 @@
     c.nffc = (pass.two_mass && pass.nmass > 2u) ? nffc.p : nullptr;
     c.bvel_zero = 1u;
     for (const BoundarySlot& b : bounds) if (b.n && (!b.vel_zero || b.sampling || b.dyn)) c.bvel_zero = 0u;
+    c.wall_regs = sw.no_wall_regs ? 0u : 1u;
     c.rho0_tab = rho0_tab.p; c.rho0_single = fluids.empty() ? 1000.0f : fluids[0].density0; c.ff_ok = ff_ok.p; c.fb_ok = fb_ok.p; c.bb_ok = bb_ok.p;
     c.partials = partials.p;
     c.spec_k = -1; c.spec_ring = spec_ring.p; c.spec_pub = nullptr; c.model_counts = model_counts.p; c.w2 = w2.p;
diff --git a/salva_amd/csrc/world_io.hip b/salva_amd/csrc/world_io.hip
--- a/salva_amd/csrc/world_io.hip
+++ b/salva_amd/csrc/world_io.hip
@@ -129,6 +129,7 @@
         case SALVA_HIP_FIELD_ACCELERATION: src = {st_acc.p, XYZ, true}; break;
         case SALVA_HIP_FIELD_DENSITY: src = {rho.p, F32, false}; break;
         case SALVA_HIP_FIELD_ALPHA: src = {alpha.p, F32, false}; break;
+        case SALVA_HIP_FIELD_KAPPA: src = {kappa.p, F32, false}; break;
         case SALVA_HIP_FIELD_NUM_FLUID_CONTACTS: src = {nff.p, U32_AS_F32, false}; break;
         case SALVA_HIP_FIELD_NUM_BOUNDARY_CONTACTS: src = {nfb.p, U32_AS_F32, false}; break;
         default: break;
diff --git a/salva_amd/world.py b/salva_amd/world.py
--- a/salva_amd/world.py
+++ b/salva_amd/world.py
@@ -1301,6 +1301,9 @@
     def pressures(self, f: Fluid) -> np.ndarray:
         return self.fluid_field(f, L.FIELD_PRESSURE)
 
+    def kappas(self, f: Fluid) -> np.ndarray:
+        return self.fluid_field(f, L.FIELD_KAPPA)
+
     def contact_counts(self, f: Fluid, boundary_contacts: bool = False) -> np.ndarray:
         fld = L.FIELD_NUM_BOUNDARY_CONTACTS if boundary_contacts else L.FIELD_NUM_FLUID_CONTACTS
         return self.fluid_field(f, fld).astype(np.uint32)
```
